# notu97/GS-SLAM-Analytica_Jacobian

Hardware: AMD Instinct MI355X
Metric: Gaussian-pixel interactions/sec (fwd+Jacobian), 640x480 (higher is better)
Workload: dtype f32; 1 GPU; cfg2: 50000 Gaussians (SH degree 3, 16 coeffs), 640x480; one step = one mapping window of 8 keyframes with distinct cameras: forward splat + analytical-Jacobian backward (dL/dmu, dL/dSigma->conic, per-Gaussian grads summed over the window, one dL/dtau per keyframe)

## Files before the change

gs-slam-analytica_jacobian_amd/csrc/api.hip:

```cpp
#include <stdarg.h>
#include <stdio.h>
#include <string.h>

#include <atomic>
#include <mutex>

#include "gsaj_common.h"
#include "loss_terms.h"

static thread_local char g_err[512] = "";

void gsaj_set_error(const char *fmt, ...) {
  va_list ap;
  va_start(ap, fmt);
  vsnprintf(g_err, sizeof(g_err), fmt, ap);
  va_end(ap);
}

struct ProfRec { int stage; hipEvent_t a, b; };
static std::mutex g_prof_mu;
static ProfRec *g_prof = nullptr;
static std::atomic<bool> g_prof_on{false};
static int g_prof_cap = 0;
static std::atomic<int> g_prof_n{0};
static thread_local int t_prof_open = -1;

void gsaj_prof_mark(int stage, int is_stop, hipStream_t s) {
  if (!g_prof_on.load(std::memory_order_acquire)) return;
  std::lock_guard<std::mutex> lk(g_prof_mu);
  if (!g_prof) return;
  if (!is_stop) {
    const int i = g_prof_n.fetch_add(1);
    if (i >= g_prof_cap) { g_prof_n.store(g_prof_cap); t_prof_open = -1; return; }
    t_prof_open = i;
    g_prof[i].stage = stage;
    (void)hipEventRecord(g_prof[i].a, s);
  } else if (t_prof_open >= 0 && t_prof_open < g_prof_cap) {
    (void)hipEventRecord(g_prof[t_prof_open].b, s);
    t_prof_open = -1;
  }
}

extern "C" {

int gsaj_profile_begin(int max_records) {
  std::lock_guard<std::mutex> lk(g_prof_mu);
  if (g_prof || max_records <= 0) {
    gsaj_set_error("gsaj_profile_begin: already active or bad size");
    return GSAJ_ERR_INVALID_ARGUMENT;
  }
  g_prof = new ProfRec[max_records];
  for (int i = 0; i < max_records; i++) {
    GSAJ_HIP_CHECK(hipEventCreate(&g_prof[i].a));
    GSAJ_HIP_CHECK(hipEventCreate(&g_prof[i].b));
  }
  g_prof_cap = max_records;
  g_prof_n.store(0);
  g_prof_on.store(true, std::memory_order_release);
  return GSAJ_OK;
}

int gsaj_profile_end(float *stage_ms, int *stage_launches) {
  if (!stage_ms || !stage_launches) {
    gsaj_set_error("gsaj_profile_end: null output");
    return GSAJ_ERR_INVALID_ARGUMENT;
  }
  g_prof_on.store(false, std::memory_order_release);
  GSAJ_HIP_CHECK(hipDeviceSynchronize());
  std::lock_guard<std::mutex> lk(g_prof_mu);
  if (!g_prof) {
    gsaj_set_error("gsaj_profile_end: not active");
    return GSAJ_ERR_INVALID_ARGUMENT;
  }
  for (int i = 0; i < ST_COUNT; i++) { stage_ms[i] = 0.f; stage_launches[i] = 0; }
  const int nrec = g_prof_n.load() < g_prof_cap ? g_prof_n.load() : g_prof_cap;
  for (int i = 0; i < nrec; i++) {
    float ms = 0.f;
    if (hipEventElapsedTime(&ms, g_prof[i].a, g_prof[i].b) == hipSuccess) {
      stage_ms[g_prof[i].stage] += ms;
      stage_launches[g_prof[i].stage] += 1;
    }
  }
  for (int i = 0; i < g_prof_cap; i++) { (void)hipEventDestroy(g_prof[i].a); (void)hipEventDestroy(g_prof[i].b); }
  delete[] g_prof;
  g_prof = nullptr;
  g_prof_cap = 0;
  g_prof_n.store(0);
  return GSAJ_OK;
}

const char *gsaj_last_error(void) { return g_err; }
int gsaj_version(void) { return 103; }

size_t gsaj_geom_workspace_bytes(int P) { return geom_carve(nullptr, (size_t)(P > 0 ? P : 0), nullptr) + 256; }
size_t gsaj_image_workspace_bytes(int W, int H) { return image_carve(nullptr, W, H, nullptr) + 256; }
size_t gsaj_binning_workspace_bytes(int R) {
  return bin_carve(nullptr, (size_t)(R > 0 ? R : 0), nullptr) + 256;
}

static char *align_base(void *p) { return reinterpret_cast<char *>(gsaj_align(reinterpret_cast<size_t>(p))); }

int gsaj_forward_preprocess(int P, int D, int M, int W, int H, const float *means3D, const float *shs,
                            const float *colors_precomp, const float *opacities, const float *scales,
                            float scale_modifier, const float *rotations, const float *cov3D_precomp,
                            const float *viewmatrix, const float *projmatrix, const float *campos, float tanfovx,
                            float tanfovy, int prefiltered, int *radii, int *n_touched, void *geom_ws, void *image_ws,
                            void *stream) {
  return gsaj_forward_preprocess_cap(P, D, M, W, H, means3D, shs, colors_precomp, opacities, scales, scale_modifier, rotations,
                                     cov3D_precomp, viewmatrix, projmatrix, campos, tanfovx, tanfovy, prefiltered, radii,
                                     n_touched, geom_ws, image_ws, 0, 0, stream);
}

int gsaj_forward_preprocess_cap(int P, int D, int M, int W, int H, const float *means3D, const float *shs,
                                const float *colors_precomp, const float *opacities, const float *scales,
                                float scale_modifier, const float *rotations, const float *cov3D_precomp,
                                const float *viewmatrix, const float *projmatrix, const float *campos, float tanfovx,
                                float tanfovy, int prefiltered, int *radii, int *n_touched, void *geom_ws, void *image_ws,
                                int capacity, int tile_list_capacity, void *stream) {
  if (P <= 0 || W <= 0 || H <= 0 || !means3D || !opacities || !viewmatrix || !projmatrix || !geom_ws || !image_ws ||
      !n_touched) {
    gsaj_set_error("gsaj_forward_preprocess: invalid argument (P=%d W=%d H=%d)", P, W, H);
    return GSAJ_ERR_INVALID_ARGUMENT;
  }
  if ((shs == nullptr) == (colors_precomp == nullptr)) {
    gsaj_set_error("Please provide excatly one of either SHs or precomputed colors!");
    return GSAJ_ERR_INVALID_ARGUMENT;
  }
  if (((scales == nullptr || rotations == nullptr) && cov3D_precomp == nullptr) ||
      ((scales != nullptr || rotations != nullptr) && cov3D_precomp != nullptr)) {
    gsaj_set_error("Please provide exactly one of either scale/rotation pair or precomputed 3D covariance!");
    return GSAJ_ERR_INVALID_ARGUMENT;
  }
  if (shs && (!campos || M <= 0 || D < 0 || (D + 1) * (D + 1) > M || D > 3)) {
    gsaj_set_error("gsaj_forward_preprocess: SH degree %d needs %d coefficients, got M=%d", D, (D + 1) * (D + 1), M);
    return GSAJ_ERR_INVALID_ARGUMENT;
  }
  GeomWS g;
  geom_carve(align_base(geom_ws), (size_t)P, &g);
  FwdParams p;
  p.P = P; p.D = D; p.M = M; p.W = W; p.H = H;
  p.means3D = means3D; p.shs = shs; p.colors_precomp = colors_precomp; p.opacities = opacities;
  p.scales = scales; p.rotations = rotations; p.cov3D_precomp = cov3D_precomp;
  p.viewmatrix = viewmatrix; p.projmatrix = projmatrix; p.campos = campos;
  p.scale_modifier = scale_modifier; p.tanfovx = tanfovx; p.tanfovy = tanfovy;
  p.focal_y = H / (2.0f * tanfovy);
  p.focal_x = W / (2.0f * tanfovx);
  p.prefiltered = prefiltered;
  p.grid_x = (W + TILE - 1) / TILE; p.grid_y = (H + TILE - 1) / TILE;
  p.capacity = capacity;
  p.sort_cap = (tile_list_capacity > 0 && tile_list_capacity < SORT_CAP) ? tile_list_capacity : SORT_CAP;
  p.views = 1;
  ImageWS im;
  image_carve(align_base(image_ws), W, H, &im);
  return launch_preprocess(p, radii ? radii : g.internal_radii, n_touched, g, im, ViewStrides{0, 0, 0}, (hipStream_t)stream);
}

int gsaj_forward_num_rendered(int W, int H, const void *image_ws, void *stream, int *num_rendered, int *max_tile_list) {
  if (W <= 0 || H <= 0 || !image_ws || !num_rendered) {
    gsaj_set_error("gsaj_forward_num_rendered: invalid argument");
    return GSAJ_ERR_INVALID_ARGUMENT;
  }
  ImageWS im;
  image_carve(align_base(const_cast<void *>(image_ws)), W, H, &im);
  uint32_t host[4] = {0, 0, 0, 0};
  GSAJ_HIP_CHECK(hipMemcpyAsync(host, im.counters, sizeof(host), hipMemcpyDeviceToHost, (hipStream_t)stream));
  GSAJ_HIP_CHECK(hipStreamSynchronize((hipStream_t)stream));
  *num_rendered = (int)host[0];
  if (max_tile_list) *max_tile_list = (int)host[2];
  if (host[1] & ERR_PREFILTERED) {
    gsaj_set_error("Point is filtered although prefiltered is set. This shouldn't happen!");
    return GSAJ_ERR_PREFILTERED_CULLED;
  }
  if (host[1] & ERR_INTERNAL) {
    gsaj_set_error("internal error: tile histogram total != instance total");
    return GSAJ_ERR_HIP;
  }
  if (host[1] & ERR_CAPACITY) {
    gsaj_set_error("async forward aborted: binning arena too small (R=%u, longest tile list=%u)", host[0], host[2]);
    return GSAJ_ERR_WORKSPACE_TOO_SMALL;
  }
  return GSAJ_OK;
}

int gsaj_forward_aborted_count(int W, int H, void *image_ws, void *stream, int *count) {
  if (W <= 0 || H <= 0 || !image_ws || !count) {
    gsaj_set_error("gsaj_forward_aborted_count: invalid argument");
    return GSAJ_ERR_INVALID_ARGUMENT;
  }
  ImageWS im;
  image_carve(align_base(image_ws), W, H, &im);
  uint32_t host = 0;
  GSAJ_HIP_CHECK(hipMemcpyAsync(&host, im.sticky, sizeof(host), hipMemcpyDeviceToHost, (hipStream_t)stream));
  GSAJ_HIP_CHECK(hipStreamSynchronize((hipStream_t)stream));
  *count = (int)host;
  if (host) GSAJ_HIP_CHECK(hipMemsetAsync(im.sticky, 0, sizeof(uint32_t), (hipStream_t)stream));
  return GSAJ_OK;
}

const uint32_t *gsaj_forward_abort_flag(int W, int H, void *image_ws) {
  if (W <= 0 || H <= 0 || !image_ws) {
    gsaj_set_error("gsaj_forward_abort_flag: invalid argument");
    return nullptr;
  }
  ImageWS im;
  image_carve(align_base(image_ws), W, H, &im);
  return im.counters + 4;
}

int gsaj_set_tile_band(int W, int H, void *image_ws, int tile_row_begin, int tile_row_end, void *stream) {
  const int gy = (H + TILE - 1) / TILE;
  if (W <= 0 || H <= 0 || !image_ws || tile_row_begin < 0 || tile_row_end < tile_row_begin || tile_row_end > gy || gy > 0xffff) {
    gsaj_set_error("gsaj_set_tile_band: rows [%d, %d) are not a band of the %d tile rows of a %dx%d frame", tile_row_begin,
                   tile_row_end, gy, W, H);
    return GSAJ_ERR_INVALID_ARGUMENT;
  }
  ImageWS im;
  image_carve(align_base(image_ws), W, H, &im);
  const bool whole = tile_row_begin == 0 && tile_row_end == gy;
  if (!whole && tile_row_end == 0) {
    gsaj_set_error("gsaj_set_tile_band: the empty band [0, 0) cannot be expressed; give an empty band as [b, b) with b > 0");
    return GSAJ_ERR_INVALID_ARGUMENT;
  }
  const uint32_t band = whole ? 0u : ((uint32_t)tile_row_begin | ((uint32_t)tile_row_end << 16));
  GSAJ_HIP_CHECK(hipMemsetD32Async(reinterpret_cast<hipDeviceptr_t>(im.sticky + 1), (int)band, 1, (hipStream_t)stream));
  GSAJ_HIP_CHECK(hipMemsetD32Async(reinterpret_cast<hipDeviceptr_t>(im.sticky + 2), (int)~band, 1, (hipStream_t)stream));
  return GSAJ_OK;
}

int gsaj_forward_render(int P, int R, int max_tile_list, int W, int H, const float *bg, const float *colors_precomp,
                        const int *radii,
                        void *geom_ws, void *binning_ws, size_t binning_ws_bytes, void *image_ws, float *out_color,
                        float *out_depth, float *out_opacity, int *n_touched, int flags, void *stream) {
  if (P <= 0 || R < 0 || W <= 0 || H <= 0 || !bg || !geom_ws || !binning_ws || !image_ws || !out_color || !out_depth ||
      !out_opacity || !n_touched) {
    gsaj_set_error("gsaj_forward_render: invalid argument");
    return GSAJ_ERR_INVALID_ARGUMENT;
  }
  const size_t need = gsaj_binning_workspace_bytes(R);
  if (binning_ws_bytes < need) {
    gsaj_set_error("binning workspace too small: have %zu bytes, need %zu for R=%d", binning_ws_bytes, need, R);
    return GSAJ_ERR_WORKSPACE_TOO_SMALL;
  }
  hipStream_t s = (hipStream_t)stream;
  GeomWS g;
  geom_carve(align_base(geom_ws), (size_t)P, &g);
  ImageWS im;
  image_carve(align_base(image_ws), W, H, &im);
  BinWS b;
  bin_carve(align_base(binning_ws), (size_t)R, &b);
  const int gx = (W + TILE - 1) / TILE, gy = (H + TILE - 1) / TILE;
  (void)colors_precomp;
  (void)radii;
  const int sort_cap = max_tile_list < 0 ? 128 : (max_tile_list > SORT_CAP ? SORT_CAP : max_tile_list);
  int rc;
  if ((rc = launch_tile_binning(P, sort_cap, (flags & GSAJ_FWD_RECORDS_FP16) ? 1 : 0, gx, gy, g, b, im, 1, ViewStrides{0, 0, 0}, s)) != GSAJ_OK) return rc;
  return launch_render_forward(P, W, H, gx, gy, bg, g, b, im, out_color, out_depth, out_opacity, n_touched, 1, ViewStrides{0, 0, 0}, s);
}

int gsaj_rasterize_forward(int P, int D, int M, const float *bg, int W, int H, const float *means3D, const float *shs,
                           const float *colors_precomp, const float *opacities, const float *scales,
                           float scale_modifier, const float *rotations, const float *cov3D_precomp,
                           const float *viewmatrix, const float *projmatrix, const float *campos, float tanfovx,
                           float tanfovy, int prefiltered, float *out_color, float *out_depth, float *out_opacity,
                           int *radii, int *n_touched, void *geom_ws, void *binning_ws, size_t binning_ws_bytes,
                           void *image_ws, int *num_rendered_out, int flags, void *stream) {
  int rc = gsaj_forward_preprocess(P, D, M, W, H, means3D, shs, colors_precomp, opacities, scales, scale_modifier,
                                   rotations, cov3D_precomp, viewmatrix, projmatrix, campos, tanfovx, tanfovy,
                                   prefiltered, radii, n_touched, geom_ws, image_ws, stream);
  if (rc != GSAJ_OK) return rc;
  int R = 0, max_tile = 0;
  rc = gsaj_forward_num_rendered(W, H, image_ws, stream, &R, &max_tile);
  if (num_rendered_out) *num_rendered_out = R;
  if (rc != GSAJ_OK) return rc;
  rc = gsaj_forward_render(P, R, max_tile, W, H, bg, colors_precomp, radii, geom_ws, binning_ws, binning_ws_bytes, image_ws,
                           out_color, out_depth, out_opacity, n_touched, flags, stream);
  return rc == GSAJ_OK ? R : rc;
}

static int forward_async_impl(int P, int D, int M, const float *bg, int W, int H, const float *means3D, const float *shs,
                              const float *colors_precomp, const float *opacities, const float *scales,
                              float scale_modifier, const float *rotations, const float *cov3D_precomp,
                              const float *viewmatrix, const float *projmatrix, const float *campos, float tanfovx,
                              float tanfovy, int prefiltered, float *out_color, float *out_depth, float *out_opacity,
                              int *radii, int *n_touched, void *geom_ws, void *binning_ws, size_t binning_ws_bytes,
                              int capacity, int tile_list_capacity, void *image_ws, int flags, void *stream, const FusedLoss *fl,
                              float *out_scalars) {
  if (capacity <= 0 || !binning_ws || !bg || !out_color || !out_depth || !out_opacity || !n_touched) {
    gsaj_set_error("gsaj_rasterize_forward_async: invalid argument");
    return GSAJ_ERR_INVALID_ARGUMENT;
  }
  if (binning_ws_bytes < gsaj_binning_workspace_bytes(capacity)) {
    gsaj_set_error("binning workspace smaller than gsaj_binning_workspace_bytes(capacity=%d)", capacity);
    return GSAJ_ERR_WORKSPACE_TOO_SMALL;
  }
  int rc = gsaj_forward_preprocess_cap(P, D, M, W, H, means3D, shs, colors_precomp, opacities, scales, scale_modifier,
                                       rotations, cov3D_precomp, viewmatrix, projmatrix, campos, tanfovx, tanfovy,
                                       prefiltered, radii, n_touched, geom_ws, image_ws, capacity, tile_list_capacity, stream);
  if (rc != GSAJ_OK) return rc;
  hipStream_t s = (hipStream_t)stream;
  GeomWS g;
  geom_carve(align_base(geom_ws), (size_t)P, &g);
  ImageWS im;
  image_carve(align_base(image_ws), W, H, &im);
  BinWS b;
  bin_carve(align_base(binning_ws), (size_t)capacity, &b);
  const int gx = (W + TILE - 1) / TILE, gy = (H + TILE - 1) / TILE;
  const int sort_cap = (tile_list_capacity > 0 && tile_list_capacity < SORT_CAP) ? tile_list_capacity : SORT_CAP;
  if ((rc = launch_tile_binning(P, sort_cap, (flags & GSAJ_FWD_RECORDS_FP16) ? 1 : 0, gx, gy, g, b, im, 1, ViewStrides{0, 0, 0}, s)) != GSAJ_OK) return rc;
  if ((rc = launch_render_forward(P, W, H, gx, gy, bg, g, b, im, out_color, out_depth, out_opacity, n_touched, 1, ViewStrides{0, 0, 0}, s, fl)) != GSAJ_OK) return rc;
  if (fl) return launch_loss_finalize(*fl, gsaj_fwd_loss_slots(W, H), W, H, im.counters + 4, out_scalars, s);
  return GSAJ_OK;
}

int gsaj_rasterize_forward_async(int P, int D, int M, const float *bg, int W, int H, const float *means3D, const float *shs,
                                 const float *colors_precomp, const float *opacities, const float *scales,
                                 float scale_modifier, const float *rotations, const float *cov3D_precomp,
                                 const float *viewmatrix, const float *projmatrix, const float *campos, float tanfovx,
                                 float tanfovy, int prefiltered, float *out_color, float *out_depth, float *out_opacity,
                                 int *radii, int *n_touched, void *geom_ws, void *binning_ws, size_t binning_ws_bytes,
                                 int capacity, int tile_list_capacity, void *image_ws, int flags, void *stream) {
  return forward_async_impl(P, D, M, bg, W, H, means3D, shs, colors_precomp, opacities, scales, scale_modifier, rotations, cov3D_precomp,
                            viewmatrix, projmatrix, campos, tanfovx, tanfovy, prefiltered, out_color, out_depth, out_opacity, radii,
                            n_touched, geom_ws, binning_ws, binning_ws_bytes, capacity, tile_list_capacity, image_ws, flags, stream,
                            nullptr, nullptr);
}

static int fused_loss_args(const char *who, int loss_flags, const float *gt_color, const float *gt_depth, const float *exposure_a,
                           const float *exposure_b) {
  const bool mono = loss_flags & GSAJ_LOSS_MONOCULAR, noexp = loss_flags & GSAJ_LOSS_NO_EXPOSURE;
  if ((loss_flags & GSAJ_LOSS_COMPUTE_LOSS) || !gt_color || (!mono && !gt_depth) || (!noexp && (!exposure_a || !exposure_b))) {
    gsaj_set_error("%s: invalid loss arguments (flags=%d; GSAJ_LOSS_COMPUTE_LOSS has no fused form)", who, loss_flags);
    return GSAJ_ERR_INVALID_ARGUMENT;
  }
  return GSAJ_OK;
}

size_t gsaj_fused_loss_workspace_bytes(int W, int H) { return (size_t)gsaj_fwd_loss_slots(W, H) * 4 * sizeof(float) + 256; }

int gsaj_rasterize_forward_loss(int P, int D, int M, const float *bg, int W, int H, const float *means3D, const float *shs,
                                const float *colors_precomp, const float *opacities, const float *scales, float scale_modifier,
                                const float *rotations, const float *cov3D_precomp, const float *viewmatrix,
                                const float *projmatrix, const float *campos, float tanfovx, float tanfovy, int prefiltered,
                                float *out_color, float *out_depth, float *out_opacity, int *radii, int *n_touched, void *geom_ws,
                                void *binning_ws, size_t binning_ws_bytes, int capacity, int tile_list_capacity, void *image_ws,
                                int flags, int loss_flags, float alpha, float rgb_boundary_threshold, const float *gt_color,
                                const float *gt_depth, const uint8_t *grad_mask, const float *exposure_a, const float *exposure_b,
                                float *out_scalars, void *loss_ws, void *stream) {
  int rc = fused_loss_args("gsaj_rasterize_forward_loss", loss_flags, gt_color, gt_depth, exposure_a, exposure_b);
  if (rc != GSAJ_OK) return rc;
  if (!out_scalars || !loss_ws) {
    gsaj_set_error("gsaj_rasterize_forward_loss: out_scalars and loss_ws are required");
    return GSAJ_ERR_INVALID_ARGUMENT;
  }
  FusedLoss fl{};
  fl.flags = loss_flags; fl.alpha = alpha; fl.rgb_thr = rgb_boundary_threshold;
  fl.gt_color = gt_color; fl.gt_depth = gt_depth; fl.grad_mask = grad_mask; fl.exp_a = exposure_a; fl.exp_b = exposure_b;
  fl.partials = reinterpret_cast<float *>(align_base(loss_ws));
  return forward_async_impl(P, D, M, bg, W, H, means3D, shs, colors_precomp, opacities, scales, scale_modifier, rotations, cov3D_precomp,
                            viewmatrix, projmatrix, campos, tanfovx, tanfovy, prefiltered, out_color, out_depth, out_opacity, radii,
                            n_touched, geom_ws, binning_ws, binning_ws_bytes, capacity, tile_list_capacity, image_ws, flags, stream, &fl,
                            out_scalars);
}

static int batch_workspaces(int K, int P, int capacity, int W, int H, void *geom_ws, void *binning_ws, size_t binning_ws_bytes,
                            void *image_ws, GeomWS *g, BinWS *b, ImageWS *im, ViewStrides *vs) {
  vs->geom = gsaj_geom_workspace_bytes(P);
  vs->image = gsaj_image_workspace_bytes(W, H);
  vs->bin = gsaj_binning_workspace_bytes(capacity);
  if (((uintptr_t)geom_ws | (uintptr_t)binning_ws | (uintptr_t)image_ws) & 255) {
    gsaj_set_error("batched entry points need 256-byte aligned workspaces");
    return GSAJ_ERR_INVALID_ARGUMENT;
  }
  if (binning_ws_bytes < vs->bin * (size_t)K) {
    gsaj_set_error("binning workspace smaller than K x gsaj_binning_workspace_bytes(capacity=%d)", capacity);
    return GSAJ_ERR_WORKSPACE_TOO_SMALL;
  }
  geom_carve(reinterpret_cast<char *>(geom_ws), (size_t)P, g);
  image_carve(reinterpret_cast<char *>(image_ws), W, H, im);
  bin_carve(reinterpret_cast<char *>(binning_ws), (size_t)capacity, b);
  return GSAJ_OK;
}

int gsaj_rasterize_forward_batch(int K, int P, int D, int M, const float *bg, int W, int H, const float *means3D, const float *shs,
                                 const float *colors_precomp, const float *opacities, const float *scales, float scale_modifier,
                                 const float *rotations, const float *cov3D_precomp, const float *viewmatrices,
                                 const float *projmatrices, const float *campos, float tanfovx, float tanfovy, int prefiltered,
                                 float *out_color, float *out_depth, float *out_opacity, int *radii, int *n_touched, void *geom_ws,
                                 void *binning_ws, size_t binning_ws_bytes, int capacity, int tile_list_capacity, void *image_ws,
                                 int flags, void *stream) {
  if (K <= 0 || P <= 0 || W <= 0 || H <= 0 || capacity <= 0 || !means3D || !opacities || !viewmatrices || !projmatrices || !bg ||
      !out_color || !out_depth || !out_opacity || !radii || !n_touched || !geom_ws || !binning_ws || !image_ws) {
    gsaj_set_error("gsaj_rasterize_forward_batch: invalid argument (K=%d P=%d W=%d H=%d capacity=%d)", K, P, W, H, capacity);
    return GSAJ_ERR_INVALID_ARGUMENT;
  }
  if ((shs == nullptr) == (colors_precomp == nullptr)) {
    gsaj_set_error("Please provide excatly one of either SHs or precomputed colors!");
    return GSAJ_ERR_INVALID_ARGUMENT;
  }
  if (((scales == nullptr || rotations == nullptr) && cov3D_precomp == nullptr) ||
      ((scales != nullptr || rotations != nullptr) && cov3D_precomp != nullptr)) {
    gsaj_set_error("Please provide exactly one of either scale/rotation pair or precomputed 3D covariance!");
    return GSAJ_ERR_INVALID_ARGUMENT;
  }
  if (shs && (!campos || M <= 0 || D < 0 || (D + 1) * (D + 1) > M || D > 3)) {
    gsaj_set_error("gsaj_rasterize_forward_batch: SH degree %d needs %d coefficients, got M=%d", D, (D + 1) * (D + 1), M);
    return GSAJ_ERR_INVALID_ARGUMENT;
  }
  GeomWS g; BinWS b; ImageWS im; ViewStrides vs;
  int rc = batch_workspaces(K, P, capacity, W, H, geom_ws, binning_ws, binning_ws_bytes, image_ws, &g, &b, &im, &vs);
  if (rc != GSAJ_OK) return rc;
  hipStream_t s = (hipStream_t)stream;
  FwdParams p;
  p.P = P; p.D = D; p.M = M; p.W = W; p.H = H;
  p.means3D = means3D; p.shs = shs; p.colors_precomp = colors_precomp; p.opacities = opacities;
  p.scales = scales; p.rotations = rotations; p.cov3D_precomp = cov3D_precomp;
  p.viewmatrix = viewmatrices; p.projmatrix = projmatrices; p.campos = campos;
  p.scale_modifier = scale_modifier; p.tanfovx = tanfovx; p.tanfovy = tanfovy;
  p.focal_y = H / (2.0f * tanfovy);
  p.focal_x = W / (2.0f * tanfovx);
  p.prefiltered = prefiltered;
  p.grid_x = (W + TILE - 1) / TILE; p.grid_y = (H + TILE - 1) / TILE;
  p.capacity = capacity;
  p.sort_cap = (tile_list_capacity > 0 && tile_list_capacity < SORT_CAP) ? tile_list_capacity : SORT_CAP;
  p.views = K;
  if ((rc = launch_preprocess(p, radii, n_touched, g, im, vs, s)) != GSAJ_OK) return rc;
  if ((rc = launch_tile_binning(P, p.sort_cap, (flags & GSAJ_FWD_RECORDS_FP16) ? 1 : 0, p.grid_x, p.grid_y, g, b, im, K, vs, s)) != GSAJ_OK)
    return rc;
  return launch_render_forward(P, W, H, p.grid_x, p.grid_y, bg, g, b, im, out_color, out_depth, out_opacity, n_touched, K, vs, s);
}

int gsaj_rasterize_backward_batch(int K, int P, int D, int M, int capacity, const float *bg, int W, int H, const float *means3D,
                                  const float *shs, const float *colors_precomp, const float *scales, float scale_modifier,
                                  const float *rotations, const float *cov3D_precomp, const float *viewmatrices,
                                  const float *projmatrices, const float *projmatrix_raw, const float *campos, float tanfovx,
                                  float tanfovy, const int *radii, void *geom_ws, void *binning_ws, void *image_ws,
                                  const float *dL_dpix, const float *dL_dpix_depth, float *dL_dmean2D, float *dL_dconic,
                                  float *dL_dopacity, float *dL_dcolor, float *dL_ddepth, float *dL_dmean3D, float *dL_dcov3D,
                                  float *dL_dsh, float *dL_dscale, float *dL_drot, float *dL_dtau, float *dL_dtau_sum, int flags,
                                  void *stream) {
  if (K <= 0 || P <= 0 || capacity <= 0 || W <= 0 || H <= 0 || !bg || !means3D || !viewmatrices || !projmatrices || !projmatrix_raw ||
      !radii || !geom_ws || !binning_ws || !image_ws || !dL_dpix || !dL_dpix_depth || !dL_dopacity || !dL_dmean3D || !dL_dcov3D ||
      !dL_dtau_sum) {
    gsaj_set_error("gsaj_rasterize_backward_batch: invalid argument");
    return GSAJ_ERR_INVALID_ARGUMENT;
  }
  if ((shs && (!dL_dsh || !campos)) || (scales && (!rotations || !dL_dscale || !dL_drot)) || (!scales && !cov3D_precomp)) {
    gsaj_set_error("gsaj_rasterize_backward_batch: missing gradient buffer for a provided input");
    return GSAJ_ERR_INVALID_ARGUMENT;
  }
  GeomWS g; BinWS b; ImageWS im; ViewStrides vs;
  int rc = batch_workspaces(K, P, capacity, W, H, geom_ws, binning_ws, gsaj_binning_workspace_bytes(capacity) * (size_t)K, image_ws,
                            &g, &b, &im, &vs);
  if (rc != GSAJ_OK) return rc;
  hipStream_t s = (hipStream_t)stream;
  const int gx = (W + TILE - 1) / TILE, gy = (H + TILE - 1) / TILE;
  const int fused = (flags & (GSAJ_BWD_ONLY_COMPOSITE | GSAJ_BWD_ONLY_CHAIN)) ? 0 : 1;
  if (!(flags & GSAJ_BWD_ONLY_CHAIN)) {
    if ((rc = launch_render_backward(capacity, W, H, gx, gy, bg, g, b, im, dL_dpix, dL_dpix_depth, K, vs, s)) != GSAJ_OK) return rc;
    if (!fused && (rc = launch_gather_sums(P, K, radii, g, b, im, vs, s)) != GSAJ_OK) return rc;
  }
  if (flags & GSAJ_BWD_ONLY_COMPOSITE) return GSAJ_OK;
  BwdParams p;
  p.P = P; p.D = D; p.M = M; p.W = W; p.H = H;
  p.means3D = means3D; p.shs = shs; p.scales = scales; p.rotations = rotations;
  p.cov3Ds = cov3D_precomp ? cov3D_precomp : g.cov3D;
  p.viewmatrix = viewmatrices; p.projmatrix = projmatrices; p.projmatrix_raw = projmatrix_raw; p.campos = campos;
  p.scale_modifier = scale_modifier; p.tanfovx = tanfovx; p.tanfovy = tanfovy;
  p.focal_y = H / (2.0f * tanfovy);
  p.focal_x = W / (2.0f * tanfovx);
  p.grid_x = gx; p.grid_y = gy;
  p.radii = radii;
  p.dL_dmean2D = dL_dmean2D; p.dL_dconic = dL_dconic; p.dL_dopacity = dL_dopacity; p.dL_dcolor = dL_dcolor;
  p.dL_ddepth = dL_ddepth; p.dL_dmean3D = dL_dmean3D; p.dL_dcov3D = dL_dcov3D; p.dL_dsh = dL_dsh;
  p.dL_dscale = dL_dscale; p.dL_drot = dL_drot; p.dL_dtau = dL_dtau; p.dL_dtau_sum = dL_dtau_sum;
  (void)colors_precomp;
  return launch_gaussian_backward_batch(p, K, g, b, im, vs, (flags & GSAJ_BWD_ACCUMULATE) ? 1 : 0, fused, s);
}

static int backward_impl(int P, int D, int M, int R, const float *bg, int W, int H, const float *means3D,
                         const float *shs, const float *colors_precomp, const float *scales, float scale_modifier,
                         const float *rotations, const float *cov3D_precomp, const float *viewmatrix,
                         const float *projmatrix, const float *projmatrix_raw, const float *campos, float tanfovx,
                         float tanfovy, const int *radii, void *geom_ws, void *binning_ws, void *image_ws,
                         const float *dL_dpix, const float *dL_dpix_depth, float *dL_dmean2D, float *dL_dconic,
                         float *dL_dopacity, float *dL_dcolor, float *dL_ddepth, float *dL_dmean3D,
                         float *dL_dcov3D, float *dL_dsh, float *dL_dscale, float *dL_drot, float *dL_dtau,
                         float *dL_dtau_sum, void *stream, const FusedLoss *fl) {
  const bool pose_only = !dL_dmean2D && !dL_dconic && !dL_dopacity && !dL_dcolor && !dL_ddepth && !dL_dmean3D && !dL_dcov3D &&
                         !dL_dsh && !dL_dscale && !dL_drot && dL_dtau_sum;
  if (P <= 0 || R < 0 || W <= 0 || H <= 0 || !bg || !means3D || !viewmatrix || !projmatrix || !projmatrix_raw ||
      !geom_ws || !binning_ws || !image_ws || (!fl && (!dL_dpix || !dL_dpix_depth)) ||
      (!pose_only && (!dL_dmean2D || !dL_dconic || !dL_dopacity || !dL_dcolor || !dL_ddepth || !dL_dmean3D || !dL_dcov3D))) {
    gsaj_set_error("gsaj_rasterize_backward: invalid argument");
    return GSAJ_ERR_INVALID_ARGUMENT;
  }
  if ((shs && ((!pose_only && !dL_dsh) || !campos)) || (scales && (!rotations || (!pose_only && (!dL_dscale || !dL_drot)))) ||
      (!scales && !cov3D_precomp)) {
    gsaj_set_error("gsaj_rasterize_backward: missing gradient buffer for a provided input");
    return GSAJ_ERR_INVALID_ARGUMENT;
  }
  hipStream_t s = (hipStream_t)stream;
  GeomWS g;
  geom_carve(align_base(geom_ws), (size_t)P, &g);
  ImageWS im;
  image_carve(align_base(image_ws), W, H, &im);
  BinWS b;
  bin_carve(align_base(binning_ws), (size_t)R, &b);
  const int gx = (W + TILE - 1) / TILE, gy = (H + TILE - 1) / TILE;
  int rc = launch_render_backward(R, W, H, gx, gy, bg, g, b, im, dL_dpix, dL_dpix_depth, 1, ViewStrides{0, 0, 0}, s, fl);
  if (rc != GSAJ_OK) return rc;
  BwdParams p;
  p.P = P; p.D = D; p.M = M; p.W = W; p.H = H;
  p.means3D = means3D; p.shs = shs; p.scales = scales; p.rotations = rotations;
  p.cov3Ds = cov3D_precomp ? cov3D_precomp : g.cov3D;
  p.viewmatrix = viewmatrix; p.projmatrix = projmatrix; p.projmatrix_raw = projmatrix_raw; p.campos = campos;
  p.scale_modifier = scale_modifier; p.tanfovx = tanfovx; p.tanfovy = tanfovy;
  p.focal_y = H / (2.0f * tanfovy);
  p.focal_x = W / (2.0f * tanfovx);
  p.grid_x = gx; p.grid_y = gy;
  p.radii = radii ? radii : g.internal_radii;
  p.dL_dmean2D = dL_dmean2D; p.dL_dconic = dL_dconic; p.dL_dopacity = dL_dopacity; p.dL_dcolor = dL_dcolor;
  p.dL_ddepth = dL_ddepth; p.dL_dmean3D = dL_dmean3D; p.dL_dcov3D = dL_dcov3D; p.dL_dsh = dL_dsh;
  p.dL_dscale = dL_dscale; p.dL_drot = dL_drot; p.dL_dtau = dL_dtau; p.dL_dtau_sum = dL_dtau_sum;
  (void)colors_precomp;
  return launch_gaussian_backward(p, g, b, im, s);
}

int gsaj_rasterize_backward(int P, int D, int M, int R, const float *bg, int W, int H, const float *means3D,
                            const float *shs, const float *colors_precomp, const float *scales, float scale_modifier,
                            const float *rotations, const float *cov3D_precomp, const float *viewmatrix,
                            const float *projmatrix, const float *projmatrix_raw, const float *campos, float tanfovx,
                            float tanfovy, const int *radii, void *geom_ws, void *binning_ws, void *image_ws,
                            const float *dL_dpix, const float *dL_dpix_depth, float *dL_dmean2D, float *dL_dconic,
                            float *dL_dopacity, float *dL_dcolor, float *dL_ddepth, float *dL_dmean3D,
                            float *dL_dcov3D, float *dL_dsh, float *dL_dscale, float *dL_drot, float *dL_dtau,
                            float *dL_dtau_sum, void *stream) {
  return backward_impl(P, D, M, R, bg, W, H, means3D, shs, colors_precomp, scales, scale_modifier, rotations, cov3D_precomp, viewmatrix,
                       projmatrix, projmatrix_raw, campos, tanfovx, tanfovy, radii, geom_ws, binning_ws, image_ws, dL_dpix, dL_dpix_depth,
                       dL_dmean2D, dL_dconic, dL_dopacity, dL_dcolor, dL_ddepth, dL_dmean3D, dL_dcov3D, dL_dsh, dL_dscale, dL_drot, dL_dtau,
                       dL_dtau_sum, stream, nullptr);
}

int gsaj_rasterize_backward_loss(int P, int D, int M, int R, const float *bg, int W, int H, const float *means3D, const float *shs,
                                 const float *colors_precomp, const float *scales, float scale_modifier, const float *rotations,
                                 const float *cov3D_precomp, const float *viewmatrix, const float *projmatrix,
                                 const float *projmatrix_raw, const float *campos, float tanfovx, float tanfovy, const int *radii,
                                 void *geom_ws, void *binning_ws, void *image_ws, int loss_flags, float alpha,
                                 float rgb_boundary_threshold, const float *color, const float *depth, const float *opacity,
                                 const float *gt_color, const float *gt_depth, const uint8_t *grad_mask, const float *exposure_a,
                                 const float *exposure_b, float *dL_dmean2D, float *dL_dconic, float *dL_dopacity, float *dL_dcolor,
                                 float *dL_ddepth, float *dL_dmean3D, float *dL_dcov3D, float *dL_dsh, float *dL_dscale,
                                 float *dL_drot, float *dL_dtau, float *dL_dtau_sum, void *stream) {
  int rc = fused_loss_args("gsaj_rasterize_backward_loss", loss_flags, gt_color, gt_depth, exposure_a, exposure_b);
  if (rc != GSAJ_OK) return rc;
  if (!color || !opacity || (!(loss_flags & GSAJ_LOSS_MONOCULAR) && !depth)) {
    gsaj_set_error("gsaj_rasterize_backward_loss: the forward's color / depth / opacity images are required");
    return GSAJ_ERR_INVALID_ARGUMENT;
  }
  FusedLoss fl{};
  fl.flags = loss_flags; fl.alpha = alpha; fl.rgb_thr = rgb_boundary_threshold;
  fl.gt_color = gt_color; fl.gt_depth = gt_depth; fl.grad_mask = grad_mask; fl.exp_a = exposure_a; fl.exp_b = exposure_b;
  fl.color = color; fl.depth = depth; fl.opacity = opacity;
  return backward_impl(P, D, M, R, bg, W, H, means3D, shs, colors_precomp, scales, scale_modifier, rotations, cov3D_precomp, viewmatrix,
                       projmatrix, projmatrix_raw, campos, tanfovx, tanfovy, radii, geom_ws, binning_ws, image_ws, nullptr, nullptr,
                       dL_dmean2D, dL_dconic, dL_dopacity, dL_dcolor, dL_ddepth, dL_dmean3D, dL_dcov3D, dL_dsh, dL_dscale, dL_drot, dL_dtau,
                       dL_dtau_sum, stream, &fl);
}

int gsaj_mark_visible(int P, const float *means3D, const float *viewmatrix, const float *projmatrix, uint8_t *present,
                      void *stream) {
  (void)projmatrix;
  if (P <= 0 || !means3D || !viewmatrix || !present) {
    gsaj_set_error("gsaj_mark_visible: invalid argument");
    return GSAJ_ERR_INVALID_ARGUMENT;
  }
  return launch_mark_visible(P, means3D, viewmatrix, present, (hipStream_t)stream);
}

int gsaj_debug_export(int P, int R, int W, int H, const void *geom_ws, const void *binning_ws, const void *image_ws,
                      float *means2D, float *depths, float *cov3D, float *conic_opacity, float *rgb, uint8_t *clamped,
                      uint32_t *tiles_touched, uint32_t *point_list, uint32_t *ranges, float *final_T,
                      uint32_t *n_contrib, void *stream) {
  hipStream_t s = (hipStream_t)stream;
  const size_t Pz = (size_t)P, N = (size_t)W * H;
  const size_t tiles = (size_t)((W + TILE - 1) / TILE) * ((H + TILE - 1) / TILE);
#define CP(dst, src, bytes) \
  if (dst) GSAJ_HIP_CHECK(hipMemcpyAsync(dst, src, bytes, hipMemcpyDeviceToDevice, s))
  if (geom_ws) {
    GeomWS g;
    geom_carve(align_base(const_cast<void *>(geom_ws)), Pz, &g);
#define CP2D(dst, src, width) \
  if (dst) GSAJ_HIP_CHECK(hipMemcpy2DAsync(dst, width, src, sizeof(float4) * REC_F4, width, Pz, hipMemcpyDeviceToDevice, s))
    CP2D(means2D, g.splat, sizeof(float2));
    CP2D(conic_opacity, g.splat + 1, sizeof(float4));
    CP2D(rgb, g.splat + 2, sizeof(float) * 3);
#undef CP2D
    CP(depths, g.depths, sizeof(float) * Pz);
    CP(cov3D, g.cov3D, sizeof(float) * 6 * Pz);
    CP(clamped, g.clamped, 3 * Pz);
    CP(tiles_touched, g.tiles_touched, sizeof(uint32_t) * Pz);
  }
  if (binning_ws && R > 0) {
    BinWS b;
    bin_carve(align_base(const_cast<void *>(binning_ws)), (size_t)R, &b);
    CP(point_list, b.point_list, sizeof(uint32_t) * (size_t)R);
  }
  if (image_ws) {
    ImageWS im;
    image_carve(align_base(const_cast<void *>(image_ws)), W, H, &im);
    CP(ranges, im.ranges, sizeof(uint2) * tiles);
    CP(final_T, im.final_T, sizeof(float) * N);
    CP(n_contrib, im.n_contrib, sizeof(uint32_t) * N);
  }
#undef CP
  return GSAJ_OK;
}

int gsaj_debug_export_view_sums(int P, const void *geom_ws, float *sums, void *stream) {
  if (P <= 0 || !geom_ws || !sums) {
    gsaj_set_error("gsaj_debug_export_view_sums: invalid argument");
    return GSAJ_ERR_INVALID_ARGUMENT;
  }
  GeomWS g;
  geom_carve(align_base(const_cast<void *>(geom_ws)), (size_t)P, &g);
  GSAJ_HIP_CHECK(hipMemcpyAsync(sums, g.gsum, sizeof(float4) * 3 * (size_t)P, hipMemcpyDeviceToDevice, (hipStream_t)stream));
  return GSAJ_OK;
}

int gsaj_debug_export_view_sums_gather(int P, int capacity, int W, int H, void *geom_ws, void *binning_ws, void *image_ws, float *sums,
                                       void *stream) {
  if (P <= 0 || capacity <= 0 || W <= 0 || H <= 0 || !geom_ws || !binning_ws || !image_ws || !sums) {
    gsaj_set_error("gsaj_debug_export_view_sums_gather: invalid argument");
    return GSAJ_ERR_INVALID_ARGUMENT;
  }
  GeomWS g; BinWS b; ImageWS im; ViewStrides vs;
  int rc = batch_workspaces(1, P, capacity, W, H, geom_ws, binning_ws, gsaj_binning_workspace_bytes(capacity), image_ws, &g, &b, &im, &vs);
  if (rc != GSAJ_OK) return rc;
  if ((rc = launch_gather_sums(P, 1, nullptr, g, b, im, vs, (hipStream_t)stream)) != GSAJ_OK) return rc;
  GSAJ_HIP_CHECK(hipMemcpyAsync(sums, g.gsum, sizeof(float4) * 3 * (size_t)P, hipMemcpyDeviceToDevice, (hipStream_t)stream));
  return GSAJ_OK;
}

}
```

gs-slam-analytica_jacobian_amd/csrc/gsaj_common.h:

```cpp
#pragma once
#include <hip/hip_runtime.h>
#include <stddef.h>
#include <stdint.h>

#include "../../include/gsaj.h"

#define GSAJ_WAVE 64
#define TILE GSAJ_TILE
#define TILE_PIXELS (TILE * TILE)
#define PRE_BLOCK 256
#define GB_BLOCK 64
#define REC_F4 3
#define IGRAD_F 12


static inline __host__ __device__ size_t gsaj_align(size_t x) { return (x + 255) & ~(size_t)255; }

struct GeomWS {
  float *depths;
  float *cov3D;
  uint8_t *clamped;
  uint32_t *tiles_touched;
  uint32_t *point_offsets;
  int *internal_radii;
  uint32_t *block_sums;
  float *tau_partials;
  float4 *splat;
  float4 *splat16;
  uint2 *scat;
  float4 *gsum;
};

static inline __host__ __device__ size_t geom_carve(char *base, size_t P, GeomWS *g) {
  size_t off = 0;
  size_t nblk = (P + PRE_BLOCK - 1) / PRE_BLOCK;
  if (nblk == 0) nblk = 1;
#define CARVE(field, type, count)                                \
  do {                                                           \
    if (g) g->field = reinterpret_cast<type *>(base + off);      \
    off += gsaj_align(sizeof(type) * (size_t)(count));           \
  } while (0)
  CARVE(depths, float, P);
  CARVE(cov3D, float, P * 6);
  CARVE(clamped, uint8_t, P * 3);
  CARVE(tiles_touched, uint32_t, P);
  CARVE(point_offsets, uint32_t, P);
  CARVE(internal_radii, int, P);
  CARVE(block_sums, uint32_t, nblk);
  CARVE(tau_partials, float, ((P + 31) / 32 + 1) * 8);
  CARVE(splat, float4, P * 3);
  CARVE(splat16, float4, P * 2);
  CARVE(scat, uint2, P);
  CARVE(gsum, float4, P * 3);
  return off;
}

#define TILE_REP 1
#define LDS_TILES_MAX 8192
#define SORT_CAP 16384
#define N_COUNTERS 64
#define ERR_PREFILTERED 1u
#define ERR_INTERNAL 2u
#define ERR_CAPACITY 4u
#define ERR_TILE_LIST 8u

struct ImageWS {
  float *final_T;
  uint32_t *n_contrib;
  uint2 *ranges;
  uint32_t *counters;
  uint32_t *tile_count;
  uint32_t *tile_cursor;
  uint32_t *tile_offset;
  uint32_t *sticky;
  uint32_t *tile_order;
  size_t zero_bytes;
};

static inline __host__ __device__ size_t image_carve(char *base, int W, int H, ImageWS *s) {
  size_t off = 0;
  size_t N = (size_t)W * H;
  size_t tiles = (size_t)((W + TILE - 1) / TILE) * ((H + TILE - 1) / TILE);
  ImageWS *g = s;
  CARVE(final_T, float, N);
  CARVE(n_contrib, uint32_t, N);
  CARVE(ranges, uint2, tiles);
  const size_t z0 = off;
  CARVE(counters, uint32_t, N_COUNTERS);
  CARVE(tile_count, uint32_t, tiles * TILE_REP);
  CARVE(tile_cursor, uint32_t, tiles * TILE_REP);
  if (g) g->zero_bytes = off - z0;
  CARVE(tile_offset, uint32_t, tiles * TILE_REP + 1);
  CARVE(sticky, uint32_t, 16);
  CARVE(tile_order, uint32_t, tiles);
  return off;
}

struct BinWS {
  uint64_t *keys_unsorted;
  uint64_t *keys;
  uint32_t *point_list;
  float4 *inst_grad;
  uint8_t *reached;
};

struct ViewStrides {
  size_t geom, image, bin;
};
#ifdef __HIPCC__
#include <type_traits>
template <typename T>
__device__ __forceinline__ T *gsaj_shift(T *p, size_t bytes) {
  typedef typename std::conditional<std::is_const<T>::value, const char, char>::type byte_t;
  return reinterpret_cast<T *>(reinterpret_cast<byte_t *>(p) + bytes);
}
__device__ __forceinline__ GeomWS geom_view(GeomWS g, size_t off) {
  g.depths = gsaj_shift(g.depths, off); g.cov3D = gsaj_shift(g.cov3D, off); g.clamped = gsaj_shift(g.clamped, off);
  g.tiles_touched = gsaj_shift(g.tiles_touched, off); g.point_offsets = gsaj_shift(g.point_offsets, off);
  g.internal_radii = gsaj_shift(g.internal_radii, off); g.block_sums = gsaj_shift(g.block_sums, off);
  g.tau_partials = gsaj_shift(g.tau_partials, off); g.splat = gsaj_shift(g.splat, off); g.gsum = gsaj_shift(g.gsum, off);
  g.splat16 = gsaj_shift(g.splat16, off); g.scat = gsaj_shift(g.scat, off);
  return g;
}
__device__ __forceinline__ ImageWS image_view(ImageWS m, size_t off) {
  m.final_T = gsaj_shift(m.final_T, off); m.n_contrib = gsaj_shift(m.n_contrib, off); m.ranges = gsaj_shift(m.ranges, off);
  m.counters = gsaj_shift(m.counters, off); m.tile_count = gsaj_shift(m.tile_count, off);
  m.tile_cursor = gsaj_shift(m.tile_cursor, off); m.tile_offset = gsaj_shift(m.tile_offset, off);
  m.sticky = gsaj_shift(m.sticky, off); m.tile_order = gsaj_shift(m.tile_order, off);
  return m;
}
#endif

static inline size_t bin_carve(char *base, size_t R, BinWS *g) {
  size_t off = 0;
  size_t Rn = R ? R : 1;
  CARVE(keys_unsorted, uint64_t, Rn);
  CARVE(keys, uint64_t, Rn);
  CARVE(point_list, uint32_t, Rn);
  CARVE(inst_grad, float4, Rn * REC_F4);
  CARVE(reached, uint8_t, Rn);
  return off;
}
#undef CARVE

void gsaj_set_error(const char *fmt, ...);
#define GSAJ_HIP_CHECK(expr)                                                          \
  do {                                                                                \
    hipError_t _e = (expr);                                                           \
    if (_e != hipSuccess) {                                                           \
      gsaj_set_error("%s failed: %s (%s:%d)", #expr, hipGetErrorString(_e), __FILE__, __LINE__); \
      return GSAJ_ERR_HIP;                                                            \
    }                                                                                 \
  } while (0)

enum GsajStage {
  ST_PREPROCESS = 0, ST_SCAN, ST_EMIT_KEYS, ST_SORT, ST_RANGES_RECORDS, ST_RENDER_FWD, ST_RENDER_BWD, ST_GAUSSIAN_BWD,
  ST_TAU_FINALIZE, ST_DENSE_BWD, ST_DENSE_REDUCE, ST_SCATTER, ST_TILE_SORT, ST_GATHER_SUMS, ST_COUNT
};
void gsaj_prof_mark(int stage, int is_stop, hipStream_t s);
struct GsajProfScope {
  int stage;
  hipStream_t s;
  GsajProfScope(int st, hipStream_t stream) : stage(st), s(stream) { gsaj_prof_mark(stage, 0, s); }
  ~GsajProfScope() { gsaj_prof_mark(stage, 1, s); }
};

struct FwdParams {
  int P, D, M, W, H;
  const float *means3D, *shs, *colors_precomp, *opacities, *scales, *rotations, *cov3D_precomp;
  const float *viewmatrix, *projmatrix, *campos;
  float scale_modifier, tanfovx, tanfovy, focal_x, focal_y;
  int prefiltered;
  int grid_x, grid_y;
  int capacity;
  int sort_cap;
  int bpw;
  int views;
};

int launch_preprocess(const FwdParams &p, int *radii, int *n_touched, const GeomWS &g, const ImageWS &im, ViewStrides vs,
                      hipStream_t s);
int launch_tile_binning(int P, int sort_cap, int rec16, int grid_x, int grid_y, const GeomWS &g, const BinWS &b, const ImageWS &im,
                        int views, ViewStrides vs, hipStream_t s);
struct FusedLoss;
int launch_render_forward(int P, int W, int H, int grid_x, int grid_y, const float *bg, const GeomWS &g, const BinWS &b,
                          const ImageWS &im, float *out_color, float *out_depth, float *out_opacity, int *n_touched, int views,
                          ViewStrides vs, hipStream_t s, const FusedLoss *fl = nullptr);
int gsaj_fwd_loss_slots(int W, int H);
int launch_loss_finalize(const FusedLoss &fl, int nslots, int W, int H, const uint32_t *aborted, float *out_scalars, hipStream_t s);
int launch_render_backward(int R, int W, int H, int grid_x, int grid_y, const float *bg, const GeomWS &g, const BinWS &b,
                           const ImageWS &im, const float *dL_dpix, const float *dL_dpix_depth, int views, ViewStrides vs,
                           hipStream_t s, const FusedLoss *fl = nullptr);
struct BwdParams {
  int P, D, M, W, H;
  const float *means3D, *shs, *scales, *rotations, *cov3Ds;
  const float *viewmatrix, *projmatrix, *projmatrix_raw, *campos;
  float scale_modifier, tanfovx, tanfovy, focal_x, focal_y;
  int grid_x, grid_y;
  const int *radii;
  float *dL_dmean2D, *dL_dconic, *dL_dopacity, *dL_dcolor, *dL_ddepth, *dL_dmean3D, *dL_dcov3D, *dL_dsh, *dL_dscale,
      *dL_drot, *dL_dtau, *dL_dtau_sum;
};
int launch_gaussian_backward(const BwdParams &p, const GeomWS &g, const BinWS &b, const ImageWS &im, hipStream_t s);
int launch_gather_sums(int P, int K, const int *radii, const GeomWS &g, const BinWS &b, const ImageWS &im, ViewStrides vs, hipStream_t s);
int launch_gaussian_backward_batch(const BwdParams &p, int K, const GeomWS &g, const BinWS &b, const ImageWS &im, ViewStrides vs,
                                   int accumulate, int gather, hipStream_t s);
int launch_mark_visible(int P, const float *means3D, const float *viewmatrix, uint8_t *present, hipStream_t s);
void launch_exclusive_scan_u32(int n, uint32_t *v, hipStream_t s);
int launch_select_rank_f32(int W, int H, const float *values, uint32_t rank, uint32_t *out_key, void *seed_ws, hipStream_t s);

#ifdef __HIPCC__
__device__ __forceinline__ float3 xform4x3(const float *m, float3 p) {
  return make_float3(m[0] * p.x + m[4] * p.y + m[8] * p.z + m[12], m[1] * p.x + m[5] * p.y + m[9] * p.z + m[13],
                     m[2] * p.x + m[6] * p.y + m[10] * p.z + m[14]);
}
__device__ __forceinline__ float4 xform4x4(const float *m, float3 p) {
  return make_float4(m[0] * p.x + m[4] * p.y + m[8] * p.z + m[12], m[1] * p.x + m[5] * p.y + m[9] * p.z + m[13],
                     m[2] * p.x + m[6] * p.y + m[10] * p.z + m[14], m[3] * p.x + m[7] * p.y + m[11] * p.z + m[15]);
}
__device__ __forceinline__ float ndc2pix(float v, int S) { return (float)((((double)v + 1.0) * (double)S - 1.0) * 0.5); }

__device__ __forceinline__ uint32_t gsaj_tile_band(const uint32_t *__restrict__ sticky) {
  const uint32_t band = sticky[1];
  return sticky[2] == ~band ? band : 0u;
}
__device__ __forceinline__ void tile_rect(float px, float py, int r, int gx, int gy, uint32_t band, int &x0, int &y0, int &x1,
                                          int &y1) {
  const int ylo = band ? (int)(band & 0xffffu) : 0, yhi = band ? min(gy, (int)(band >> 16)) : gy;
  x0 = min(gx, max(0, (int)((px - (float)r) / (float)TILE)));
  y0 = min(yhi, max(ylo, (int)((py - (float)r) / (float)TILE)));
  x1 = min(gx, max(0, (int)((px + (float)r + (float)(TILE - 1)) / (float)TILE)));
  y1 = min(yhi, max(ylo, (int)((py + (float)r + (float)(TILE - 1)) / (float)TILE)));
}
#define GSAJ_LOG2E 1.4426950408889634f
__device__ __forceinline__ float3 gsaj_prescale_conic(float a, float b, float c) {
  return make_float3((-0.5f * GSAJ_LOG2E) * a, -GSAJ_LOG2E * b, (-0.5f * GSAJ_LOG2E) * c);
}
__device__ __forceinline__ float gsaj_power2(float dx, float dy, float kx, float ky, float kz) {
  const float t = ky * dy;
  const float u = kz * dy;
  return __builtin_fmaf(dx, __builtin_fmaf(kx, dx, t), u * dy);
}
__device__ __forceinline__ float3 cross3(float3 a, float3 b) {
  return make_float3(a.y * b.z - a.z * b.y, a.z * b.x - a.x * b.z, a.x * b.y - a.y * b.x);
}
#endif

#define REC16_F4 2
#ifdef __HIPCC__
#include <hip/hip_fp16.h>
__device__ __forceinline__ uint32_t gsaj_pack_h2(float a, float b) {
  const __half2 h = __floats2half2_rn(a, b);
  return *reinterpret_cast<const uint32_t *>(&h);
}
__device__ __forceinline__ float2 gsaj_unpack_h2(uint32_t u) { return __half22float2(*reinterpret_cast<const __half2 *>(&u)); }
__device__ __forceinline__ void gsaj_load_row(const float4 *__restrict__ splat, const float4 *__restrict__ splat16, uint32_t id,
                                              bool rec16, float4 &q0, float4 &q1, float4 &q2) {
  if (!rec16) {
    const float4 *s = splat + (size_t)id * REC_F4;
    const float4 r0 = s[0], r1 = s[1], r2 = s[2];
    q0 = make_float4(r0.x, r0.y, r2.w, r0.w);
    q1 = r1;
    q2 = make_float4(r2.x, r2.y, r2.z, r0.z);
    return;
  }
  const float4 *s = splat16 + (size_t)id * REC16_F4;
  const float4 p0 = s[0], p1 = s[1];
  const float2 ab = gsaj_unpack_h2(__float_as_uint(p1.x)), co = gsaj_unpack_h2(__float_as_uint(p1.y));
  const float2 rg = gsaj_unpack_h2(__float_as_uint(p1.z)), bz = gsaj_unpack_h2(__float_as_uint(p1.w));
  q0 = p0;
  q1 = make_float4(ab.x, ab.y, co.x, co.y);
  q2 = make_float4(rg.x, rg.y, bz.x, 0.f);
}
#endif

#ifdef __HIPCC__
__device__ __forceinline__ float4 gsaj_load_f4_unaligned(const void *src) {
  typedef float f4u __attribute__((ext_vector_type(4), aligned(4)));
  const f4u v = *reinterpret_cast<const __attribute__((address_space(1))) f4u *>((unsigned long long)src);
  return make_float4(v.x, v.y, v.z, v.w);
}
__device__ __forceinline__ uint32_t gsaj_load_u32_global(const uint32_t *src) {
  return *reinterpret_cast<const __attribute__((address_space(1))) uint32_t *>((unsigned long long)src);
}
__device__ __forceinline__ uint4 gsaj_coherent_load_x4(const void *src) {
  uint4 v;
  asm volatile("global_load_dwordx4 %0, %1, off sc0 sc1\n\ts_waitcnt vmcnt(0)" : "=&v"(v) : "v"(src) : "memory");
  return v;
}
#endif

#ifdef GSAJ_BLOCK_TRACE
#define GSAJ_TRACE_MAX 65536
#define GSAJ_TRACE_DEFINE(NAME)                                                                               \
  __device__ unsigned long long g_trace_##NAME[4 * GSAJ_TRACE_MAX];                                           \
  extern "C" int gsaj_trace_read_##NAME(unsigned long long *host, int nwaves) {                               \
    return (int)hipMemcpyFromSymbol(host, HIP_SYMBOL(g_trace_##NAME), sizeof(unsigned long long) * 4 * nwaves); \
  }
#define GSAJ_TRACE_BEGIN(NAME)                                                                                \
  {                                                                                                           \
    const unsigned tw_ = (blockIdx.y * gridDim.x + blockIdx.x) * (blockDim.x >> 6) + (threadIdx.x >> 6);      \
    if ((threadIdx.x & 63) == 0 && tw_ < GSAJ_TRACE_MAX) {                                                    \
      g_trace_##NAME[4 * tw_ + 0] = wall_clock64();                                                           \
      g_trace_##NAME[4 * tw_ + 2] = __builtin_amdgcn_s_getreg((4) | (0 << 6) | (31 << 11));                   \
      g_trace_##NAME[4 * tw_ + 3] = __builtin_amdgcn_s_getreg((20) | (0 << 6) | (31 << 11));                  \
    }                                                                                                         \
  }
#define GSAJ_TRACE_END(NAME)                                                                                  \
  {                                                                                                           \
    const unsigned tw_ = (blockIdx.y * gridDim.x + blockIdx.x) * (blockDim.x >> 6) + (threadIdx.x >> 6);      \
    if ((threadIdx.x & 63) == 0 && tw_ < GSAJ_TRACE_MAX) g_trace_##NAME[4 * tw_ + 1] = wall_clock64();        \
  }
#else
#define GSAJ_TRACE_DEFINE(NAME)
#define GSAJ_TRACE_BEGIN(NAME)
#define GSAJ_TRACE_END(NAME)
#endif
```

gs-slam-analytica_jacobian_amd/csrc/render_bwd.hip:

```cpp
#include "gsaj_common.h"
#include "loss_terms.h"
#include "wave_reduce.h"

#define BWD_ROUND 48
#define SLOTS 8
#define WU_STRIDE 65
#define ACC_C 10
#define ACC_STRIDE (BWD_ROUND + 1)

GSAJ_TRACE_DEFINE(bwd)
GSAJ_TRACE_DEFINE(bwdph)
#ifdef GSAJ_BLOCK_TRACE
#define BWD_PH(i) { const unsigned long long now_ = wall_clock64(); ph_[i] += (unsigned)(now_ - pht_); pht_ = now_; }
#else
#define BWD_PH(i)
#endif

template <bool LOSS>
__global__ __launch_bounds__(256) __attribute__((amdgpu_waves_per_eu(5, 5))) void k_render_bwd(int W, int H, int gx, ImageWS im,
                                                    const uint32_t *__restrict__ point_list, GeomWS g,
                                                    const float *__restrict__ bg,
                                                    const float *__restrict__ dL_dpix,
                                                    const float *__restrict__ dL_dpix_depth,
                                                    float4 *__restrict__ inst_grad, uint8_t *__restrict__ reached, ViewStrides vs,
                                                    FusedLoss fl) {
  {
    const size_t view = blockIdx.y, HWv = (size_t)H * W;
    im = image_view(im, view * vs.image);
    point_list = gsaj_shift(point_list, view * vs.bin);
    g = geom_view(g, view * vs.geom);
    inst_grad = gsaj_shift(inst_grad, view * vs.bin);
    reached = gsaj_shift(reached, view * vs.bin);
    dL_dpix += view * 3 * HWv;
    dL_dpix_depth += view * HWv;
  }
  const uint2 *__restrict__ ranges = im.ranges;
  const float *__restrict__ final_T = im.final_T;
  const uint32_t *__restrict__ n_contrib = im.n_contrib;
  const uint32_t *__restrict__ counters = im.counters;
  __shared__ float4 rec[BWD_ROUND * REC_F4];
  __shared__ __attribute__((aligned(16))) float acc[4 * ACC_C * ACC_STRIDE];
  __shared__ float2 wu_all[4 * SLOTS * WU_STRIDE];
  __shared__ float4 seed_all[4 * 64];
  __shared__ uint32_t wave_max[4];
  __shared__ uint32_t blk_first[BWD_ROUND];
  if (counters[4]) return;
  GSAJ_TRACE_BEGIN(bwd)
  const int tid = threadIdx.x, wave = tid >> 6, lane = tid & 63;
  float2 *wu = wu_all + wave * SLOTS * WU_STRIDE;
  float4 *seed = seed_all + wave * 64;
  const int tile = __builtin_amdgcn_readfirstlane((int)min(im.tile_order[blockIdx.x], gridDim.x - 1));
  const int ty = tile / gx, tx = tile - ty * gx;
  const int px = tx * TILE + (wave & 1) * 8 + (lane & 7);
  const int py = ty * TILE + (wave >> 1) * 8 + (lane >> 3);
  const bool inside = px < W && py < H;
  const float pxf = (float)px, pyf = (float)py;
  const float qx0 = (float)(tx * TILE + (wave & 1) * 8), qy0 = (float)(ty * TILE + (wave >> 1) * 8);
  const uint2 range_v = ranges[tile];
  const uint2 range = make_uint2((uint32_t)__builtin_amdgcn_readfirstlane((int)range_v.x), (uint32_t)__builtin_amdgcn_readfirstlane((int)range_v.y));
  const size_t pid = (size_t)py * W + px, HW = (size_t)H * W;

  const float T_final = inside ? final_T[pid] : 0.f;
  float T = T_final;
  const uint32_t last = inside ? n_contrib[pid] : 0u;
  float gC0 = 0.f, gC1 = 0.f, gC2 = 0.f, gD = 0.f;
  if (inside) {
    if (LOSS) {
      const LossConsts L = loss_consts(fl.flags, fl.alpha, fl.rgb_thr, fl.exp_a, fl.exp_b, HW, 1.f);
      const bool mask = fl.grad_mask ? fl.grad_mask[pid] != 0 : true;
      const float gd = L.mono ? 0.f : fl.gt_depth[pid], d = L.mono ? 0.f : fl.depth[pid];
      const LossPixel o = loss_pixel(L, fl.gt_color[pid], fl.gt_color[HW + pid], fl.gt_color[2 * HW + pid], fl.color[pid], fl.color[HW + pid],
                                     fl.color[2 * HW + pid], fl.opacity[pid], mask, gd, d);
      gC0 = o.gC0; gC1 = o.gC1; gC2 = o.gC2; gD = o.gD;
    } else {
      gC0 = dL_dpix[pid];
      gC1 = dL_dpix[HW + pid];
      gC2 = dL_dpix[2 * HW + pid];
      gD = dL_dpix_depth[pid];
    }
  }
  seed[lane] = make_float4(gC0, gC1, gC2, gD);
  const float Tf_bg = T_final * (bg[0] * gC0 + bg[1] * gC1 + bg[2] * gC2);
  const float ddelx_dx = 0.5f * W, ddely_dy = 0.5f * H;

  uint32_t wmax = last;
#pragma unroll
  for (int o = 32; o > 0; o >>= 1) wmax = max(wmax, (uint32_t)__shfl_xor((int)wmax, o));
  if (lane == 0) wave_max[wave] = wmax;
  __syncthreads();
  const uint32_t bmax = max(max(wave_max[0], wave_max[1]), max(wave_max[2], wave_max[3]));

  float accS = 0.f;

  const int p2_slot = lane & (SLOTS - 1), p2_row = lane >> 3;
  const float p2_py = qy0 + (float)p2_row;

  uint32_t hi = (uint32_t)__builtin_amdgcn_readfirstlane((int)(range.x + bmax));
  const bool rec16 = counters[7] != 0u;
  const int part = __builtin_amdgcn_readfirstlane(wave), e = lane;
  auto round_lo = [&](uint32_t h) { return (h - range.x > BWD_ROUND) ? h - BWD_ROUND : range.x; };
  auto load_id = [&](uint32_t l, uint32_t h) -> uint32_t {
    const bool has = e < BWD_ROUND && l + (uint32_t)e < h;
    const uint32_t v = gsaj_load_u32_global(point_list + (has ? l + (uint32_t)e : range.x));
    return has ? v : 0xffffffffu;
  };
  const char *piece_base;
  uint32_t piece_stride;
  if (part == 3) piece_base = reinterpret_cast<const char *>(g.block_sums), piece_stride = 0u;
  else if (!rec16) piece_base = reinterpret_cast<const char *>(g.splat + part), piece_stride = 16u * REC_F4;
  else if (part < 2) piece_base = reinterpret_cast<const char *>(g.splat16 + part), piece_stride = 16u * REC16_F4;
  else piece_base = reinterpret_cast<const char *>(g.scat), piece_stride = 8u;
  auto load_piece = [&](uint32_t id) -> float4 {
    const uint32_t i = id != 0xffffffffu ? id : 0u;
    const size_t off = piece_stride ? (size_t)i * piece_stride : (size_t)(i / PRE_BLOCK) * 4u;
    return gsaj_load_f4_unaligned(piece_base + off);
  };
  uint32_t id_cur = 0xffffffffu, id_nxt = 0xffffffffu;
  float4 piece = make_float4(0.f, 0.f, 0.f, 0.f);
  if (hi > range.x) {
    const uint32_t lo0 = round_lo(hi);
    id_cur = load_id(lo0, hi);
    id_nxt = load_id(round_lo(lo0), lo0);
    piece = load_piece(id_cur);
  }

#ifdef GSAJ_BLOCK_TRACE
  unsigned ph_[7] = {0u, 0u, 0u, 0u, 0u, 0u, 0u};
  unsigned tr_flushes = 0u, tr_slots = 0u;
  unsigned long long pht_ = wall_clock64();
#endif
  while (hi > range.x) {
    BWD_PH(6)
    const uint32_t lo = round_lo(hi);
    const int n = (int)(hi - lo);
    if (e < n) {
      int e_ = e;
      asm volatile("" : "+v"(e_));
      const int e = e_;
      if (part == 3) {
        blk_first[e] = __float_as_uint(piece.x);
      } else if (!rec16) {
        if (part == 1) {
          const float3 kq = gsaj_prescale_conic(piece.x, piece.y, piece.z);
          rec[e * REC_F4 + 1] = make_float4(kq.x, kq.y, kq.z, piece.w);
        } else {
          rec[e * REC_F4 + part] = piece;
        }
      } else {
        float *r = reinterpret_cast<float *>(rec + e * REC_F4);
        if (part == 0) {
          r[0] = piece.x, r[1] = piece.y, r[3] = piece.w, r[11] = piece.z;
        } else if (part == 1) {
          const float2 ab = gsaj_unpack_h2(__float_as_uint(piece.x)), co = gsaj_unpack_h2(__float_as_uint(piece.y));
          const float2 rg = gsaj_unpack_h2(__float_as_uint(piece.z)), bz = gsaj_unpack_h2(__float_as_uint(piece.w));
          const float3 kq = gsaj_prescale_conic(ab.x, ab.y, co.x);
          rec[e * REC_F4 + 1] = make_float4(kq.x, kq.y, kq.z, co.y);
          r[8] = rg.x, r[9] = rg.y, r[10] = bz.x;
        } else if (part == 2) {
          const uint32_t sx = __float_as_uint(piece.x), sy = __float_as_uint(piece.y);
          const uint32_t x0 = sx & 0xffffu, y0 = sy & 0xffffu, w = (sx >> 16) - x0;
          r[2] = __uint_as_float(x0 | (y0 << 10) | (w << 20));
        }
      }
    }
    {
      const uint32_t lo2 = round_lo(lo);
      id_cur = id_nxt;
      id_nxt = load_id(round_lo(lo2), lo2);
      piece = load_piece(id_cur);
    }
    {
      float4 *z = reinterpret_cast<float4 *>(acc);
      for (int i = tid; i < 4 * ACC_C * ACC_STRIDE / 4; i += 256) z[i] = make_float4(0.f, 0.f, 0.f, 0.f);
    }
    BWD_PH(0)
    __syncthreads();
    BWD_PH(1)

    const uint32_t first_idx = (uint32_t)__builtin_amdgcn_readfirstlane((int)(lo - range.x));
    if (wmax > first_idx) {
      bool rel = false;
      if (lane < n && first_idx + (uint32_t)lane < wmax) {
        const float4 q0 = rec[lane * REC_F4 + 0];
        const float4 q1 = rec[lane * REC_F4 + 1];
        rel = quadrant_relevant(q0.x, q0.y, (-2.0f / GSAJ_LOG2E) * q1.x, (-1.0f / GSAJ_LOG2E) * q1.y, (-2.0f / GSAJ_LOG2E) * q1.z, q1.w, qx0, qy0);
      }
      unsigned long long todo = __builtin_amdgcn_ballot_w64(rel);
      int nslot = 0;
      unsigned long long slot_pack = 0ull;

      auto flush = [&]() {
#ifdef GSAJ_BLOCK_TRACE
        tr_flushes++;
        tr_slots += (unsigned)nslot;
#endif
        const int j = (int)((slot_pack >> (8 * p2_slot)) & 0xffull);
        const float4 e0 = rec[j * REC_F4 + 0];
        float4 e1 = rec[j * REC_F4 + 1];
        e1.x *= -2.0f / GSAJ_LOG2E; e1.y *= -1.0f / GSAJ_LOG2E; e1.z *= -2.0f / GSAJ_LOG2E;
        const float ax0 = e0.x - qx0, dy = e0.y - p2_py;
        float m0 = 0.f, swdx = 0.f, swdx2 = 0.f, u0 = 0.f, u1 = 0.f, u2 = 0.f, u3 = 0.f;
#pragma unroll
        for (int it = 0; it < 8; it++) {
          const int pix = p2_row * 8 + it;
          const float2 q = wu[p2_slot * WU_STRIDE + pix];
          const float4 sd = seed[pix];
          const float dx = ax0 - (float)it;
          const float wd = q.x * dx;
          m0 += q.x;
          swdx += wd;
          swdx2 = __builtin_fmaf(wd, dx, swdx2);
          u0 += q.y * sd.x;
          u1 += q.y * sd.y;
          u2 += q.y * sd.z;
          u3 += q.y * sd.w;
        }
        const float swdy = dy * m0;
        float v[10];
        v[0] = -(e1.x * swdx + e1.y * swdy) * ddelx_dx;
        v[1] = -(e1.z * swdy + e1.y * swdx) * ddely_dy;
        v[2] = -0.5f * swdx2;
        v[3] = -0.5f * (dy * swdx);
        v[4] = -0.5f * (dy * swdy);
        v[5] = m0 * __builtin_amdgcn_rcpf(e1.w);
        v[6] = u0; v[7] = u1; v[8] = u2; v[9] = u3;
        const float w0 = merge32(v[0], v[1]), w1 = merge32(v[2], v[3]), w2 = merge32(v[4], v[5]), w3 = merge32(v[6], v[7]),
                    w4 = merge32(v[8], v[9]);
        float x0 = merge16(w0, w1), x1 = merge16(w2, w3), x2 = merge16(w4, w4);
        x0 = dpp_add<0x128>(x0);
        x1 = dpp_add<0x128>(x1);
        x2 = dpp_add<0x128>(x2);
        if (p2_slot < nslot && (lane & 8) == 0) {
          const int r = lane >> 4;
          const int k = ((r & 1) << 1) | (r >> 1);
          float *a = acc + wave * ACC_C * ACC_STRIDE + j;
          a[k * ACC_STRIDE] = x0;
          a[(4 + k) * ACC_STRIDE] = x1;
          if ((r & 1) == 0) a[(8 + (r >> 1)) * ACC_STRIDE] = x2;
        }
        nslot = 0;
        slot_pack = 0ull;
      };

      if (todo != 0ull) {
        int jj = 63 - __builtin_clzll(todo);
        todo &= ~(1ull << jj);
        float2 q01 = reinterpret_cast<const float2 *>(rec)[jj * (REC_F4 * 2)];
        float4 k = rec[jj * REC_F4 + 1], c = rec[jj * REC_F4 + 2];
        while (true) {
          const int j = jj;
          const uint32_t idx = first_idx + (uint32_t)j;
          const bool more = todo != 0ull;
          if (more) {
            jj = 63 - __builtin_clzll(todo);
            todo &= ~(1ull << jj);
          }
          const float dx = q01.x - pxf, dy = q01.y - pyf;
          const float p2 = gsaj_power2(dx, dy, k.x, k.y, k.z);
          const float oG = k.w * __builtin_amdgcn_exp2f(p2);
          q01 = reinterpret_cast<const float2 *>(rec)[jj * (REC_F4 * 2)];
          k = rec[jj * REC_F4 + 1];
          const bool valid = idx < last && p2 <= 0.0f && oG >= (1.0f / 255.0f);
          float cg = __builtin_fmaf(c.x, gC0, __builtin_fmaf(c.y, gC1, __builtin_fmaf(c.z, gC2, c.w * gD)));
          asm volatile("" : "+v"(cg));
          c = rec[jj * REC_F4 + 2];
          if (__builtin_amdgcn_ballot_w64(valid) != 0ull) {
            const float oGm = valid ? oG : 0.f;
            float alpha;
            asm("v_min_f32 %0, 0x3f7d70a4, %1" : "=v"(alpha) : "v"(oGm));
            const float inv1ma = __builtin_amdgcn_rcpf(1.f - alpha);
            T = T * inv1ma;
            asm volatile("" : "+v"(T));
            const float dd = cg - accS;
            const float dL_dalpha = dd * T - Tf_bg * inv1ma;
            accS += alpha * dd;
            float w_ = dL_dalpha * oGm;
            asm volatile("" : "+v"(w_));
            wu[nslot * WU_STRIDE + lane] = make_float2(w_, alpha * T);
            slot_pack |= (unsigned long long)j << (8 * nslot);
            nslot++;
            if (nslot == SLOTS) flush();
          }
          if (!more) break;
        }
        if (nslot > 0) flush();
      }
    }
    BWD_PH(2)
    __syncthreads();
    BWD_PH(3)
    if (part < 3 && e < n) {
      float t[4];
#pragma unroll
      for (int c = 0; c < 4; c++) {
        const float *a = acc + min(part * 4 + c, ACC_C - 1) * ACC_STRIDE + e;
        t[c] = ((a[0] + a[ACC_C * ACC_STRIDE]) + a[2 * ACC_C * ACC_STRIDE]) + a[3 * ACC_C * ACC_STRIDE];
      }
      if (part == 2) t[2] = t[3] = 0.f;
      const float4 q0 = rec[e * REC_F4 + 0];
      const uint32_t rp = __float_as_uint(q0.z);
      const uint32_t x0 = rp & 1023u, y0 = (rp >> 10) & 1023u, w = rp >> 20;
      const uint32_t emit = blk_first[e] + __float_as_uint(q0.w) + ((uint32_t)ty - y0) * w + ((uint32_t)tx - x0);
      inst_grad[(size_t)emit * REC_F4 + part] = make_float4(t[0], t[1], t[2], t[3]);
      if (part == 0) reached[emit] = 1;
    }
    BWD_PH(4)
    __syncthreads();
    BWD_PH(5)
    hi = lo;
  }
#ifdef GSAJ_BLOCK_TRACE
  {
    const unsigned tw_ = (blockIdx.y * gridDim.x + blockIdx.x) * 4 + (threadIdx.x >> 6);
    if ((threadIdx.x & 63) == 0 && tw_ < GSAJ_TRACE_MAX) {
      g_trace_bwdph[4 * tw_ + 0] = ((unsigned long long)ph_[0] << 32) | ph_[1];
      g_trace_bwdph[4 * tw_ + 1] = ((unsigned long long)ph_[2] << 32) | ph_[3];
      g_trace_bwdph[4 * tw_ + 2] = ((unsigned long long)ph_[4] << 32) | ph_[5];
      g_trace_bwdph[4 * tw_ + 3] = ph_[6] | ((unsigned long long)tr_flushes << 32) | ((unsigned long long)tr_slots << 44);
    }
  }
#endif
  GSAJ_TRACE_END(bwd)
}

int launch_render_backward(int R, int W, int H, int grid_x, int grid_y, const float *bg, const GeomWS &g, const BinWS &b,
                           const ImageWS &im, const float *dL_dpix, const float *dL_dpix_depth, int views, ViewStrides vs,
                           hipStream_t s, const FusedLoss *fl) {
  if (R <= 0) return GSAJ_OK;
  {
    GsajProfScope ps(ST_RENDER_BWD, s);
    if (fl)
      hipLaunchKernelGGL(k_render_bwd<true>, dim3(grid_x * grid_y, 1), dim3(256), 0, s, W, H, grid_x, im, b.point_list, g, bg, dL_dpix,
                         dL_dpix_depth, b.inst_grad, b.reached, vs, *fl);
    else
      hipLaunchKernelGGL(k_render_bwd<false>, dim3(grid_x * grid_y, views), dim3(256), 0, s, W, H, grid_x, im, b.point_list, g, bg, dL_dpix,
                         dL_dpix_depth, b.inst_grad, b.reached, vs, FusedLoss{});
  }
  GSAJ_HIP_CHECK(hipGetLastError());
  return GSAJ_OK;
}
```

gs-slam-analytica_jacobian_amd/csrc/render_fwd.hip:

```cpp
#include "gsaj_common.h"
#include "loss_terms.h"
#include "wave_reduce.h"

#define FWD_CHUNK 64
#define FWD_PAD 8
#define FWD_PAIR_F4 6
typedef float v2f __attribute__((ext_vector_type(2)));

#ifndef GSAJ_FWD_THREADS
#define GSAJ_FWD_THREADS 64
#endif
#define FWD_WAVES (GSAJ_FWD_THREADS / 64)

GSAJ_TRACE_DEFINE(fwd)

template <bool LOSS>
__global__ __launch_bounds__(GSAJ_FWD_THREADS) __attribute__((amdgpu_waves_per_eu(5, 8))) void k_render_fwd(int W, int H, int gx, int tiles, int P, ImageWS im,
                                                    const float4 *__restrict__ splat, const float4 *__restrict__ splat16,
                                                    const float *__restrict__ bg,
                                                    float *__restrict__ out_color, float *__restrict__ out_depth,
                                                    float *__restrict__ out_opacity, int *__restrict__ n_touched,
                                                    const uint32_t *__restrict__ point_list, ViewStrides vs, FusedLoss fl) {
  {
    const size_t view = blockIdx.y, HWv = (size_t)H * W;
    im = image_view(im, view * vs.image);
    splat = gsaj_shift(splat, view * vs.geom);
    splat16 = gsaj_shift(splat16, view * vs.geom);
    point_list = gsaj_shift(point_list, view * vs.bin);
    out_color += view * 3 * HWv;
    out_depth += view * HWv;
    out_opacity += view * HWv;
    n_touched += view * (size_t)P;
  }
  const uint2 *__restrict__ ranges = im.ranges;
  float *__restrict__ final_T = im.final_T;
  uint32_t *__restrict__ n_contrib = im.n_contrib;
  uint32_t *__restrict__ counters = im.counters;
  __shared__ float4 rec_all[FWD_WAVES * ((FWD_CHUNK + FWD_PAD) / 2) * FWD_PAIR_F4];
  if (counters[4]) return;
  GSAJ_TRACE_BEGIN(fwd)
  const int tid = threadIdx.x, lane = tid & 63;
#if FWD_WAVES == 1
  const int wave = ((int)blockIdx.x >> 3) & 3;
  const int rank = ((int)blockIdx.x >> 5) * 8 + ((int)blockIdx.x & 7);
  if (rank >= tiles) {
    if (LOSS && lane == 0) reinterpret_cast<float4 *>(fl.partials)[blockIdx.x] = make_float4(0.f, 0.f, 0.f, 0.f);
    return;
  }
  const int tile = (int)min(im.tile_order[rank], (uint32_t)(tiles - 1));
  float4 *rec = rec_all;
#else
  const int wave = tid >> 6;
  const int tile = (int)min(im.tile_order[blockIdx.x], (uint32_t)(tiles - 1));
  float4 *rec = rec_all + wave * ((FWD_CHUNK + FWD_PAD) / 2) * FWD_PAIR_F4;
#endif
  const int ty = tile / gx, tx = tile - ty * gx;
  const int px = tx * TILE + (wave & 1) * 8 + (lane & 7);
  const int py = ty * TILE + (wave >> 1) * 8 + (lane >> 3);
  const bool inside = px < W && py < H;
  const float pxf = (float)px, pyf = (float)py;
  const float qx0 = (float)(tx * TILE + (wave & 1) * 8), qy0 = (float)(ty * TILE + (wave >> 1) * 8);
  const uint2 range = ranges[tile];

  bool done = !inside;
  float T = 1.0f;
  uint32_t last = 0;
  bool counting = true;

  v2f Crg = {0.f, 0.f}, Cbd = {0.f, 0.f};
  const v2f px2 = {pxf, pxf}, py2 = {pyf, pyf};
  auto composite2 = [&](const float4 p0, const float4 p1, const float4 p2, const float4 cA, const float4 cB, const float2 pos,
                        float &T_afterA) {
    const v2f dx = v2f{p0.x, p0.y} - px2, dy = v2f{p0.z, p0.w} - py2;
    const v2f t = v2f{p1.z, p1.w} * dy;
    const v2f u = v2f{p2.x, p2.y} * dy;
    const v2f pw = __builtin_elementwise_fma(dx, __builtin_elementwise_fma(v2f{p1.x, p1.y}, dx, t), u * dy);
    const v2f oe = v2f{p2.z, p2.w} * v2f{__builtin_amdgcn_exp2f(pw.x), __builtin_amdgcn_exp2f(pw.y)};
    {
      const float alpha0 = fminf(0.99f, oe.x);
      bool ok = !done && pw.x <= 0.0f && alpha0 >= (1.0f / 255.0f);
      const float tA = __builtin_fmaf(-alpha0, T, T);
      const bool sat = ok && tA < 0.0001f;
      done = done || sat;
      ok = ok && !sat;
      const float w = ok ? alpha0 * T : 0.f;
      const v2f w2 = {w, w};
      Crg = __builtin_elementwise_fma(v2f{cA.x, cA.y}, w2, Crg);
      Cbd = __builtin_elementwise_fma(v2f{cA.z, cA.w}, w2, Cbd);
      T = ok ? tA : T;
      last = ok ? __float_as_uint(pos.x) : last;
      T_afterA = T;
    }
    {
      const float alpha0 = fminf(0.99f, oe.y);
      bool ok = !done && pw.y <= 0.0f && alpha0 >= (1.0f / 255.0f);
      const float tB = __builtin_fmaf(-alpha0, T, T);
      const bool sat = ok && tB < 0.0001f;
      done = done || sat;
      ok = ok && !sat;
      const float w = ok ? alpha0 * T : 0.f;
      const v2f w2 = {w, w};
      Crg = __builtin_elementwise_fma(v2f{cB.x, cB.y}, w2, Crg);
      Cbd = __builtin_elementwise_fma(v2f{cB.z, cB.w}, w2, Cbd);
      T = ok ? tB : T;
      last = ok ? __float_as_uint(pos.y) : last;
    }
  };

  if (__builtin_amdgcn_ballot_w64(!done) != 0ull && range.x < range.y) {
    float4 q0, q1, q2;
    uint32_t id_cur = 0u, id_nxt = 0u;
    const bool rec16 = counters[7] != 0u;
    auto fetch_id = [&](uint32_t base) {
      if (base + (uint32_t)lane < range.y) id_nxt = point_list[base + lane];
    };
    auto fetch_row = [&](uint32_t base) {
      id_cur = id_nxt;
      if (base + (uint32_t)lane < range.y) gsaj_load_row(splat, splat16, id_nxt, rec16, q0, q1, q2);
    };
    float *recf = reinterpret_cast<float *>(rec);
    for (int i = lane; i < ((FWD_CHUNK + FWD_PAD) / 2) * FWD_PAIR_F4; i += 64) rec[i] = make_float4(0.f, 0.f, 0.f, 0.f);
    auto put = [&](int s, float x, float y, float kx, float ky, float kz, float o, float4 c, uint32_t pos, uint32_t id) {
      const int h = s & 1, pb = (s >> 1) * FWD_PAIR_F4;
      float *f = recf + pb * 4 + h;
      f[0] = x; f[2] = y; f[4] = kx; f[6] = ky; f[8] = kz; f[10] = o;
      rec[pb + 3 + h] = c;
      f[20] = __uint_as_float(pos); f[22] = __uint_as_float(id);
    };
    fetch_id(range.x);
    fetch_row(range.x);
    fetch_id(range.x + FWD_CHUNK);
    for (uint32_t base = range.x; base < range.y; base += FWD_CHUNK) {
      const int m = min((uint32_t)FWD_CHUNK, range.y - base);
      bool rel = false;
      const uint32_t id_here = id_cur;
      if (lane < m) rel = quadrant_relevant(q0.x, q0.y, q1.x, q1.y, q1.z, q1.w, qx0, qy0);
      const unsigned long long todo = __builtin_amdgcn_ballot_w64(rel);
      const int nrel = __popcll(todo);
      __builtin_amdgcn_wave_barrier();
      if (rel) {
        const int slot = __builtin_amdgcn_mbcnt_hi((uint32_t)(todo >> 32), __builtin_amdgcn_mbcnt_lo((uint32_t)todo, 0u));
        const float3 k = gsaj_prescale_conic(q1.x, q1.y, q1.z);
        put(slot, q0.x, q0.y, k.x, k.y, k.z, q1.w, make_float4(q2.x, q2.y, q2.z, q0.z), base - range.x + (uint32_t)lane + 1u, id_here);
      }
      if (lane < FWD_PAD) recf[((nrel + lane) >> 1) * FWD_PAIR_F4 * 4 + 10 + ((nrel + lane) & 1)] = 0.f;
      fetch_row(base + FWD_CHUNK);
      fetch_id(base + 2 * FWD_CHUNK);
      __builtin_amdgcn_fence(__ATOMIC_RELEASE, "wavefront");
      __builtin_amdgcn_wave_barrier();
      __builtin_amdgcn_fence(__ATOMIC_ACQUIRE, "wavefront");
      uint32_t cnt4 = 0u;
      bool wave_done = false;
      const float2 *rec2 = reinterpret_cast<const float2 *>(rec);
      float4 a0 = rec[0], a1 = rec[1], a2 = rec[2], a3 = rec[3], a4 = rec[4];
      float2 a5 = rec2[10];
      for (int i = 0; i < nrel; i += 4) {
        const int pb = (i >> 1) * FWD_PAIR_F4;
        const float4 c0 = rec[pb + 6], c1 = rec[pb + 7], c2 = rec[pb + 8], c3 = rec[pb + 9], c4 = rec[pb + 10];
        const float2 c5 = rec2[(pb + 11) * 2];
        uint32_t pack = 0u;
        {
          const float T0 = T;
          float Ta;
          composite2(a0, a1, a2, a3, a4, a5, Ta);
          if (counting) {
            const unsigned long long hB = __builtin_amdgcn_ballot_w64(T > 0.5f);
            const uint32_t nA = (uint32_t)__popcll(__builtin_amdgcn_ballot_w64(Ta > 0.5f) & __builtin_amdgcn_ballot_w64(Ta < T0));
            const uint32_t nB = (uint32_t)__popcll(hB & __builtin_amdgcn_ballot_w64(T < Ta));
            pack = nA | (nB << 8);
            counting = hB != 0ull;
          }
        }
        asm volatile("" : "+v"(T), "+v"(last), "+v"(Crg), "+v"(Cbd) : : "memory");
        a0 = rec[pb + 12], a1 = rec[pb + 13], a2 = rec[pb + 14], a3 = rec[pb + 15], a4 = rec[pb + 16];
        a5 = rec2[(pb + 17) * 2];
        {
          const float T0 = T;
          float Tc;
          composite2(c0, c1, c2, c3, c4, c5, Tc);
          if (counting) {
            const unsigned long long hD = __builtin_amdgcn_ballot_w64(T > 0.5f);
            const uint32_t nC = (uint32_t)__popcll(__builtin_amdgcn_ballot_w64(Tc > 0.5f) & __builtin_amdgcn_ballot_w64(Tc < T0));
            const uint32_t nD = (uint32_t)__popcll(hD & __builtin_amdgcn_ballot_w64(T < Tc));
            pack |= (nC << 16) | (nD << 24);
            counting = hD != 0ull;
          }
        }
        cnt4 = ((lane >> 2) == (i >> 2)) ? pack : cnt4;
        if (__builtin_amdgcn_ballot_w64(!done) == 0ull) {
          wave_done = true;
          break;
        }
      }
      const int cnt = (int)((cnt4 >> (8 * (lane & 3))) & 0xffu);
      if (lane < nrel && cnt > 0) {
        const uint32_t id = __float_as_uint(recf[(lane >> 1) * FWD_PAIR_F4 * 4 + 22 + (lane & 1)]);
        atomicAdd(&n_touched[id], cnt);
      }
      __builtin_amdgcn_wave_barrier();
      if (wave_done) break;
    }
  }

  const float Cr = Crg.x, Cg = Crg.y, Cb = Cbd.x, Dp = Cbd.y;
  if (inside) {
    const size_t pid = (size_t)py * W + px;
    const size_t HW = (size_t)H * W;
    final_T[pid] = T;
    n_contrib[pid] = last;
    out_color[pid] = Cr + T * bg[0];
    out_color[HW + pid] = Cg + T * bg[1];
    out_color[2 * HW + pid] = Cb + T * bg[2];
    out_depth[pid] = Dp;
    out_opacity[pid] = 1.f - T;
  }
  if (LOSS) {
    float s4[4] = {0.f, 0.f, 0.f, 0.f};
    if (inside) {
      const size_t pid = (size_t)py * W + px, HW = (size_t)H * W;
      const LossConsts L = loss_consts(fl.flags, fl.alpha, fl.rgb_thr, fl.exp_a, fl.exp_b, HW, 1.f);
      const bool mask = fl.grad_mask ? fl.grad_mask[pid] != 0 : true;
      const float gd = L.mono ? 0.f : fl.gt_depth[pid];
      const LossPixel o = loss_pixel(L, fl.gt_color[pid], fl.gt_color[HW + pid], fl.gt_color[2 * HW + pid], Cr + T * bg[0], Cg + T * bg[1],
                                     Cb + T * bg[2], 1.f - T, mask, gd, Dp);
      s4[0] = o.s_rgb; s4[1] = o.s_d; s4[2] = o.s_a; s4[3] = o.s_b;
    }
#pragma unroll
    for (int c = 0; c < 4; c++) {
#pragma unroll
      for (int o2 = 32; o2 > 0; o2 >>= 1) s4[c] += __shfl_xor(s4[c], o2);
    }
    if (lane == 0) reinterpret_cast<float4 *>(fl.partials)[blockIdx.x] = make_float4(s4[0], s4[1], s4[2], s4[3]);
  }
  GSAJ_TRACE_END(fwd)
}

int gsaj_fwd_loss_slots(int W, int H) {
  const int tiles = ((W + TILE - 1) / TILE) * ((H + TILE - 1) / TILE);
  return FWD_WAVES == 1 ? ((tiles + 7) / 8) * 32 : tiles;
}

int launch_render_forward(int P, int W, int H, int grid_x, int grid_y, const float *bg, const GeomWS &g, const BinWS &b,
                          const ImageWS &im, float *out_color, float *out_depth, float *out_opacity, int *n_touched, int views,
                          ViewStrides vs, hipStream_t s, const FusedLoss *fl) {
  static_assert(FWD_WAVES == 1, "the loss-fused epilogue writes one partial per wave-sized workgroup");
  {
    GsajProfScope ps(ST_RENDER_FWD, s);
    const int tiles = grid_x * grid_y;
    const unsigned nblk = FWD_WAVES == 1 ? (unsigned)((tiles + 7) / 8) * 32u : (unsigned)tiles;
    if (fl)
      hipLaunchKernelGGL(k_render_fwd<true>, dim3(nblk, 1), dim3(GSAJ_FWD_THREADS), 0, s, W, H, grid_x, tiles, P, im, g.splat, g.splat16, bg,
                         out_color, out_depth, out_opacity, n_touched, b.point_list, vs, *fl);
    else
      hipLaunchKernelGGL(k_render_fwd<false>, dim3(nblk, views), dim3(GSAJ_FWD_THREADS), 0, s, W, H, grid_x, tiles, P, im, g.splat, g.splat16,
                         bg, out_color, out_depth, out_opacity, n_touched, b.point_list, vs, FusedLoss{});
  }
  GSAJ_HIP_CHECK(hipGetLastError());
  return GSAJ_OK;
}
```

gs-slam-analytica_jacobian_amd/gsaj/_lib.py:

```python
import ctypes
import os
import subprocess

_HERE = os.path.dirname(os.path.abspath(__file__))
PKG_ROOT = os.path.dirname(_HERE)
CSRC = os.path.join(PKG_ROOT, "csrc")
LIB_PATH = os.environ.get("GSAJ_LIB_PATH") or os.path.join(PKG_ROOT, "lib", "libgsaj_hip.so")
HEADER = os.path.join(os.path.dirname(PKG_ROOT), "include", "gsaj.h")

c_int, c_float, c_double, c_size_t, c_void_p = ctypes.c_int, ctypes.c_float, ctypes.c_double, ctypes.c_size_t, ctypes.c_void_p
P = c_void_p

SIGNATURES = {
    "gsaj_last_error": (ctypes.c_char_p, []),
    "gsaj_version": (c_int, []),
    "gsaj_geom_workspace_bytes": (c_size_t, [c_int]),
    "gsaj_image_workspace_bytes": (c_size_t, [c_int, c_int]),
    "gsaj_binning_workspace_bytes": (c_size_t, [c_int]),
    "gsaj_forward_preprocess": (c_int, [c_int] * 5 + [P, P, P, P, P, c_float, P, P, P, P, P, c_float, c_float, c_int, P, P, P, P, P]),
    "gsaj_forward_num_rendered": (c_int, [c_int, c_int, P, P, ctypes.POINTER(c_int), ctypes.POINTER(c_int)]),
    "gsaj_forward_render": (c_int, [c_int] * 5 + [P, P, P, P, P, c_size_t, P, P, P, P, P, c_int, P]),
    "gsaj_rasterize_forward": (c_int, [c_int, c_int, c_int, P, c_int, c_int, P, P, P, P, P, c_float, P, P, P, P, P,
                                       c_float, c_float, c_int, P, P, P, P, P, P, P, c_size_t, P,
                                       ctypes.POINTER(c_int), c_int, P]),
    "gsaj_rasterize_forward_async": (c_int, [c_int, c_int, c_int, P, c_int, c_int, P, P, P, P, P, c_float, P, P, P, P, P,
                                             c_float, c_float, c_int, P, P, P, P, P, P, P, c_size_t, c_int, c_int, P, c_int, P]),
    "gsaj_rasterize_forward_batch": (c_int, [c_int, c_int, c_int, c_int, P, c_int, c_int, P, P, P, P, P, c_float, P, P, P, P, P,
                                             c_float, c_float, c_int, P, P, P, P, P, P, P, c_size_t, c_int, c_int, P, c_int, P]),
    "gsaj_rasterize_backward_batch": (c_int, [c_int, c_int, c_int, c_int, c_int, P, c_int, c_int, P, P, P, P, c_float, P, P, P, P,
                                              P, P, c_float, c_float, P, P, P, P, P, P] + [P] * 12 + [c_int, P]),
    "gsaj_fused_loss_workspace_bytes": (c_size_t, [c_int, c_int]),
    "gsaj_rasterize_forward_loss": (c_int, [c_int, c_int, c_int, P, c_int, c_int, P, P, P, P, P, c_float, P, P, P, P, P,
                                            c_float, c_float, c_int, P, P, P, P, P, P, P, c_size_t, c_int, c_int, P, c_int,
                                            c_int, c_float, c_float, P, P, P, P, P, P, P, P]),
    "gsaj_rasterize_backward_loss": (c_int, [c_int, c_int, c_int, c_int, P, c_int, c_int, P, P, P, P, c_float, P, P, P, P, P, P,
                                             c_float, c_float, P, P, P, P, c_int, c_float, c_float, P, P, P, P, P, P, P, P] + [P] * 12 + [P]),
    "gsaj_forward_aborted_count": (c_int, [c_int, c_int, P, P, ctypes.POINTER(c_int)]),
    "gsaj_set_tile_band": (c_int, [c_int, c_int, P, c_int, c_int, P]),
    "gsaj_forward_preprocess_cap": (c_int, [c_int] * 5 + [P, P, P, P, P, c_float, P, P, P, P, P, c_float, c_float, c_int, P, P,
                                            P, P, c_int, c_int, P]),
    "gsaj_rasterize_backward": (c_int, [c_int, c_int, c_int, c_int, P, c_int, c_int, P, P, P, P, c_float, P, P, P, P, P, P,
                                        c_float, c_float, P, P, P, P, P, P] + [P] * 12 + [P]),
    "gsaj_mark_visible": (c_int, [c_int, P, P, P, P, P]),
    "gsaj_debug_export": (c_int, [c_int] * 4 + [P] * 3 + [P] * 11 + [P]),
    "gsaj_debug_export_view_sums": (c_int, [c_int, P, P, P]),
    "gsaj_debug_export_view_sums_gather": (c_int, [c_int, c_int, c_int, c_int, P, P, P, P, P]),
    "gsaj_profile_begin": (c_int, [c_int]),
    "gsaj_profile_end": (c_int, [P, P]),
    "gsaj_dense_workspace_bytes": (c_size_t, [c_int, c_int, c_int]),
    "gsaj_dense_backward": (c_int, [c_int, c_int, c_int] + [P] * 7 + [P] * 4 + [P, c_int, P, P]),
    "gsaj_dense_project_workspace_bytes": (c_size_t, [c_int]),
    "gsaj_dense_project": (c_int, [c_int] * 5 + [P] * 6 + [c_double, c_double] + [P] * 6 + [P, P]),
    "gsaj_dense_render": (c_int, [c_int, c_int, c_int] + [P] * 5 + [P, P, P]),
    "gsaj_pose_jacobians": (c_int, [c_int, P, P, P, c_double, c_double, c_int, c_int, P, P, P]),
    "gsaj_dense_tau": (c_int, [c_int, c_int, c_int] + [P] * 11 + [P, P, P]),
    "gsaj_dist2_workspace_bytes": (c_size_t, [c_int]),
    "gsaj_dist2": (c_int, [c_int, P, P, P, P]),
    "gsaj_debug_dist2_order": (c_int, [c_int, P, P, P, P]),
    "gsaj_pose_state_floats": (c_int, []),
    "gsaj_pose_adam_step": (c_int, [P, P] + [c_float] * 8 + [P, P, P, P]),
    "gsaj_pose_adam_step_batch": (c_int, [c_int, P, P, P] + [c_float] * 8 + [P, P, P, c_size_t, P]),
    "gsaj_forward_abort_flag": (c_void_p, [c_int, c_int, P]),
    "gsaj_loss_workspace_bytes": (c_size_t, [c_int, c_int]),
    "gsaj_densification_stats": (c_int, [c_int, c_int] + [P] * 7 + [P]),
    "gsaj_isotropic_workspace_bytes": (c_size_t, [c_int]),
    "gsaj_isotropic_loss": (c_int, [c_int, c_int, c_float, P, P, c_int, P, P, P]),
    "gsaj_loss_seeds": (c_int, [c_int, c_int, c_int, c_float, c_float] + [P] * 8 + [P] * 4 + [P, P]),
    "gsaj_loss_seeds_batch": (c_int, [c_int] + [c_int, c_int, c_int, c_float, c_float] + [P] * 8 + [P] * 4 + [P, P]),
    "gsaj_ssim_workspace_bytes": (c_size_t, [c_int] * 4),
    "gsaj_ssim_forward": (c_int, [c_int] * 4 + [P] * 6),
    "gsaj_ssim_backward": (c_int, [c_int] * 4 + [P] * 6),
    "gsaj_refine_loss_workspace_bytes": (c_size_t, [c_int, c_int]),
    "gsaj_refine_loss_seeds": (c_int, [c_int, c_int, c_float] + [P] * 6),
    "gsaj_seed_workspace_bytes": (c_size_t, [c_int, c_int]),
    "gsaj_depth_stats": (c_int, [c_int, c_int, P, P, c_float, P, P, c_float, P, P, P, P]),
    "gsaj_keyframe_depth_prior": (c_int, [c_int, c_int, P, P, P, c_float, P, P, P, P, P]),
    "gsaj_seed_select": (c_int, [c_int, c_int, P, P, c_float, c_float, c_double, ctypes.c_uint32, P, P]),
    "gsaj_seed_count": (c_int, [P, P, ctypes.POINTER(c_int), ctypes.POINTER(c_int)]),
    "gsaj_debug_seed_pixels": (c_int, [c_int, c_int, c_int, P, P, P]),
    "gsaj_seed_gaussians": (c_int, [c_int, c_int, c_int, P, P, P, P] + [c_double] * 4 + [c_float, c_int, c_int, c_int] + [P] * 6 + [P, P, P]),
    "gsaj_grad_mask_workspace_bytes": (c_size_t, [c_int, c_int]),
    "gsaj_grad_intensity": (c_int, [c_int, c_int, P, P, P]),
    "gsaj_grad_mask": (c_int, [c_int, c_int, P, c_float, c_int, P, P, P, P]),
    "gsaj_covis_pack": (c_int, [c_int, c_int, P, ctypes.POINTER(c_int), ctypes.c_uint32, P, P]),
    "gsaj_covis_query": (c_int, [c_int, P, P, c_int, ctypes.c_uint32, P, P]),
    "gsaj_covis_prune_mask": (c_int, [c_int, P, ctypes.c_uint32, P, c_int, c_int, P, P, P, P]),
}

_lib = None


def build(verbose=False):
    cmd = ["make", "-C", CSRC, "-j8"]
    if not verbose:
        cmd.append("-s")
    subprocess.check_call(cmd)
    return LIB_PATH


def load():
    global _lib
    if _lib is not None:
        return _lib
    if not os.path.exists(LIB_PATH):
        raise ImportError(
            "libgsaj_hip.so is missing (%s). Build the HIP extension first: "
            "`python __graft_entry__.py` or `make -C %s`. There is no CPU fallback." % (LIB_PATH, CSRC))
    import torch
    lib = ctypes.CDLL(LIB_PATH)
    for name, (res, args) in SIGNATURES.items():
        fn = getattr(lib, name)
        fn.restype = res
        fn.argtypes = args
    _lib = lib
    return lib


class GsajError(RuntimeError):
    pass


def check(rc, what):
    if rc < 0:
        msg = load().gsaj_last_error().decode("utf-8", "replace")
        if rc == -1:
            raise Exception(msg or ("%s: invalid argument" % what))
        raise GsajError("%s failed (%d): %s" % (what, rc, msg))
    return rc
```

gs-slam-analytica_jacobian_amd/gsaj/rasterizer.py:

```python
import ctypes
import os

import torch

from . import _lib

_F32 = torch.float32
FORCE_CHUNKED_SORT = bool(int(__import__("os").environ.get("GSAJ_FORCE_CHUNKED_SORT", "0")))
SORT_CAP = 16384


def _ptr(t):
    if t is None or t.numel() == 0:
        return None
    return t.data_ptr()


def _prep(t, device, name):
    if t is None or t.numel() == 0:
        return None
    if t.device != device:
        t = t.to(device)
    if t.dtype != _F32:
        t = t.to(_F32)
    return t.contiguous()


def _stream(device):
    return torch.cuda.current_stream(device).cuda_stream


def _require_cuda(t, what):
    if not t.is_cuda:
        raise RuntimeError("%s must live on the GPU (HIP device): libgsaj_hip has no CPU path" % what)


def rasterize_gaussians(background, means3D, colors, opacity, scales, rotations, scale_modifier, cov3D_precomp,
                        viewmatrix, projmatrix, projmatrix_raw, tan_fovx, tan_fovy, image_height, image_width, sh,
                        degree, campos, prefiltered, debug, record_bits=32):
    lib = _lib.load()
    if means3D.ndim != 2 or means3D.shape[1] != 3:
        raise RuntimeError("means3D must have dimensions (num_points, 3)")
    _require_cuda(means3D, "means3D")
    dev = means3D.device
    P, H, W = means3D.shape[0], int(image_height), int(image_width)
    f = dict(device=dev, dtype=_F32)
    out_color = torch.zeros((3, H, W), **f)
    out_depth = torch.zeros((1, H, W), **f)
    out_opacity = torch.zeros((1, H, W), **f)
    radii = torch.zeros((P,), device=dev, dtype=torch.int32)
    n_touched = torch.zeros((P,), device=dev, dtype=torch.int32)
    byte = dict(device=dev, dtype=torch.uint8)
    if P == 0:
        e = torch.empty(0, **byte)
        return 0, out_color, radii, e, e.clone(), e.clone(), out_depth, out_opacity, n_touched

    means3D = _prep(means3D, dev, "means3D")
    colors = _prep(colors, dev, "colors")
    opacity = _prep(opacity, dev, "opacity")
    scales = _prep(scales, dev, "scales")
    rotations = _prep(rotations, dev, "rotations")
    cov3D_precomp = _prep(cov3D_precomp, dev, "cov3D")
    sh = _prep(sh, dev, "sh")
    background = _prep(background, dev, "bg")
    viewmatrix = _prep(viewmatrix, dev, "viewmatrix")
    projmatrix = _prep(projmatrix, dev, "projmatrix")
    campos = _prep(campos, dev, "campos")
    M = 0 if sh is None else sh.shape[1]

    geom = torch.empty(lib.gsaj_geom_workspace_bytes(P), **byte)
    img = torch.empty(lib.gsaj_image_workspace_bytes(W, H), **byte)
    st = _stream(dev)
    with torch.cuda.device(dev):
        _lib.check(lib.gsaj_forward_preprocess(
            P, int(degree), M, W, H, _ptr(means3D), _ptr(sh), _ptr(colors), _ptr(opacity), _ptr(scales),
            float(scale_modifier), _ptr(rotations), _ptr(cov3D_precomp), _ptr(viewmatrix), _ptr(projmatrix),
            _ptr(campos), float(tan_fovx), float(tan_fovy), int(bool(prefiltered)), radii.data_ptr(),
            n_touched.data_ptr(), geom.data_ptr(), img.data_ptr(), st), "gsaj_forward_preprocess")
        R, mt = ctypes.c_int(0), ctypes.c_int(0)
        _lib.check(lib.gsaj_forward_num_rendered(W, H, img.data_ptr(), st, ctypes.byref(R), ctypes.byref(mt)),
                   "gsaj_forward_num_rendered")
        R = R.value
        nbytes = lib.gsaj_binning_workspace_bytes(R)
        binning = torch.empty(nbytes, **byte)
        _lib.check(lib.gsaj_forward_render(
            P, R, -1 if FORCE_CHUNKED_SORT else mt.value, W, H, _ptr(background), _ptr(colors), radii.data_ptr(), geom.data_ptr(), binning.data_ptr(), nbytes,
            img.data_ptr(), out_color.data_ptr(), out_depth.data_ptr(), out_opacity.data_ptr(), n_touched.data_ptr(),
            _fwd_flags(record_bits), st), "gsaj_forward_render")
        if debug:
            torch.cuda.synchronize(dev)
    return R, out_color, radii, geom, binning, img, out_depth, out_opacity, n_touched


def rasterize_gaussians_backward(background, means3D, radii, colors, scales, rotations, scale_modifier, cov3D_precomp,
                                 viewmatrix, projmatrix, projmatrix_raw, tan_fovx, tan_fovy, dL_dout_color,
                                 dL_dout_depths, sh, degree, campos, geomBuffer, R, binningBuffer, imageBuffer, debug,
                                 per_gaussian_tau=True):
    lib = _lib.load()
    _require_cuda(means3D, "means3D")
    dev = means3D.device
    P = means3D.shape[0]
    H, W = dL_dout_color.shape[1], dL_dout_color.shape[2]
    sh = _prep(sh, dev, "sh")
    M = 0 if sh is None else sh.shape[1]
    f = dict(device=dev, dtype=_F32)
    dL_dmeans3D = torch.empty((P, 3), **f)
    dL_dmeans2D = torch.empty((P, 3), **f)
    dL_dcolors = torch.empty((P, 3), **f)
    dL_ddepths = torch.empty((P, 1), **f)
    dL_dconic = torch.empty((P, 2, 2), **f)
    dL_dopacity = torch.empty((P, 1), **f)
    dL_dcov3D = torch.empty((P, 6), **f)
    dL_dsh = torch.empty((P, M, 3), **f)
    dL_dscales = torch.empty((P, 3), **f)
    dL_drotations = torch.empty((P, 4), **f)
    dL_dtau = torch.empty((P, 6), **f) if per_gaussian_tau else None
    dL_dtau_sum = torch.zeros((6,), **f)
    if P == 0:
        return (dL_dmeans2D, dL_dcolors, dL_dopacity, dL_dmeans3D, dL_dcov3D, dL_dsh, dL_dscales, dL_drotations,
                dL_dtau, dL_dtau_sum, dL_dconic, dL_ddepths)
    means3D = _prep(means3D, dev, "means3D")
    colors = _prep(colors, dev, "colors")
    scales = _prep(scales, dev, "scales")
    rotations = _prep(rotations, dev, "rotations")
    cov3D_precomp = _prep(cov3D_precomp, dev, "cov3D")
    background = _prep(background, dev, "bg")
    viewmatrix = _prep(viewmatrix, dev, "viewmatrix")
    projmatrix = _prep(projmatrix, dev, "projmatrix")
    projmatrix_raw = _prep(projmatrix_raw, dev, "projmatrix_raw")
    campos = _prep(campos, dev, "campos")
    dL_dout_color = _prep(dL_dout_color, dev, "dL_dout_color")
    dL_dout_depths = _prep(dL_dout_depths, dev, "dL_dout_depths")
    st = _stream(dev)
    with torch.cuda.device(dev):
        _lib.check(lib.gsaj_rasterize_backward(
            P, int(degree), M, int(R), _ptr(background), W, H, _ptr(means3D), _ptr(sh), _ptr(colors), _ptr(scales),
            float(scale_modifier), _ptr(rotations), _ptr(cov3D_precomp), _ptr(viewmatrix), _ptr(projmatrix),
            _ptr(projmatrix_raw), _ptr(campos), float(tan_fovx), float(tan_fovy), radii.data_ptr(),
            geomBuffer.data_ptr(), binningBuffer.data_ptr(), imageBuffer.data_ptr(), _ptr(dL_dout_color),
            _ptr(dL_dout_depths), dL_dmeans2D.data_ptr(), dL_dconic.data_ptr(), dL_dopacity.data_ptr(),
            dL_dcolors.data_ptr(), dL_ddepths.data_ptr(), dL_dmeans3D.data_ptr(), dL_dcov3D.data_ptr(),
            _ptr(dL_dsh), _ptr(dL_dscales) if scales is not None else None,
            _ptr(dL_drotations) if rotations is not None else None,
            dL_dtau.data_ptr() if dL_dtau is not None else None, dL_dtau_sum.data_ptr(), st), "gsaj_rasterize_backward")
        if debug:
            torch.cuda.synchronize(dev)
    if scales is None:
        dL_dscales.zero_()
        dL_drotations.zero_()
    return (dL_dmeans2D, dL_dcolors, dL_dopacity, dL_dmeans3D, dL_dcov3D, dL_dsh, dL_dscales, dL_drotations, dL_dtau,
            dL_dtau_sum, dL_dconic, dL_ddepths)


def mark_visible(means3D, viewmatrix, projmatrix):
    lib = _lib.load()
    _require_cuda(means3D, "means3D")
    dev = means3D.device
    P = means3D.shape[0]
    present = torch.zeros((P,), device=dev, dtype=torch.bool)
    if P != 0:
        means3D = _prep(means3D, dev, "means3D")
        viewmatrix = _prep(viewmatrix, dev, "viewmatrix")
        projmatrix = _prep(projmatrix, dev, "projmatrix")
        with torch.cuda.device(dev):
            _lib.check(lib.gsaj_mark_visible(P, _ptr(means3D), _ptr(viewmatrix), _ptr(projmatrix), present.data_ptr(),
                                             _stream(dev)), "gsaj_mark_visible")
    return present


def debug_export(P, R, W, H, geomBuffer, binningBuffer, imageBuffer):
    lib = _lib.load()
    dev = geomBuffer.device
    tiles = ((W + 15) // 16) * ((H + 15) // 16)
    f = dict(device=dev, dtype=_F32)
    out = dict(
        means2D=torch.zeros((P, 2), **f), depths=torch.zeros((P,), **f), cov3D=torch.zeros((P, 6), **f),
        conic_opacity=torch.zeros((P, 4), **f), rgb=torch.zeros((P, 3), **f),
        clamped=torch.zeros((P, 3), device=dev, dtype=torch.uint8),
        tiles_touched=torch.zeros((P,), device=dev, dtype=torch.int32),
        point_list=torch.zeros((max(R, 1),), device=dev, dtype=torch.int32),
        ranges=torch.zeros((tiles, 2), device=dev, dtype=torch.int32), final_T=torch.zeros((H, W), **f),
        n_contrib=torch.zeros((H, W), device=dev, dtype=torch.int32))
    with torch.cuda.device(dev):
        _lib.check(lib.gsaj_debug_export(
            P, R, W, H, geomBuffer.data_ptr(), binningBuffer.data_ptr(), imageBuffer.data_ptr(),
            out["means2D"].data_ptr(), out["depths"].data_ptr(), out["cov3D"].data_ptr(),
            out["conic_opacity"].data_ptr(), out["rgb"].data_ptr(), out["clamped"].data_ptr(),
            out["tiles_touched"].data_ptr(), out["point_list"].data_ptr(), out["ranges"].data_ptr(),
            out["final_T"].data_ptr(), out["n_contrib"].data_ptr(), _stream(dev)), "gsaj_debug_export")
    out["point_list"] = out["point_list"][:R]
    return out


STAGE_NAMES = ("preprocess,scan_blocks,emit_keys,sort,ranges_records,render_fwd,render_bwd,gaussian_bwd,tau_finalize,"
               "dense_bwd,dense_reduce,scatter_instances,tile_sort_records,gather_sums").split(",")


class profile_stages:

    def __init__(self, max_records=4096):
        self.max_records = max_records
        self.ms, self.launches = {}, {}

    def __enter__(self):
        _lib.check(_lib.load().gsaj_profile_begin(self.max_records), "gsaj_profile_begin")
        return self

    def __exit__(self, *exc):
        n = len(STAGE_NAMES)
        ms = (ctypes.c_float * n)()
        cnt = (ctypes.c_int * n)()
        _lib.check(_lib.load().gsaj_profile_end(ctypes.cast(ms, ctypes.c_void_p), ctypes.cast(cnt, ctypes.c_void_p)),
                   "gsaj_profile_end")
        self.ms = {k: float(ms[i]) for i, k in enumerate(STAGE_NAMES)}
        self.launches = {k: int(cnt[i]) for i, k in enumerate(STAGE_NAMES)}
        return False


FWD_RECORDS_FP16 = 1


def _fwd_flags(record_bits):
    if record_bits not in (16, 32):
        raise ValueError("record_bits must be 16 or 32, got %r" % (record_bits,))
    return FWD_RECORDS_FP16 if record_bits == 16 else 0


class ArenaWatch:

    def __init__(self, img, K, img_stride, counters_offset, every=4, grow_at=0.75):
        self.K, self.every, self.grow_at = int(K), int(every), float(grow_at)
        i32 = img.view(torch.int32)
        self.dev_counters = torch.as_strided(i32, (self.K, 4), (img_stride // 4, 1), counters_offset // 4)
        self.host = torch.zeros((self.K, 4), dtype=torch.int32).pin_memory()
        self.event = torch.cuda.Event()
        self.pending, self.calls = False, 0
        self.grown = 0
        with torch.cuda.device(img.device):
            self.host.copy_(self.dev_counters, non_blocking=True)
            self.event.record()
            self.event.synchronize()

    def post(self):
        self.calls += 1
        if self.pending or self.calls % self.every or torch.cuda.is_current_stream_capturing():
            return
        self.host.copy_(self.dev_counters, non_blocking=True)
        self.event.record()
        self.pending = True

    def poll(self):
        if not self.pending or torch.cuda.is_current_stream_capturing() or not self.event.query():
            return None
        self.pending = False
        return int(self.host[:, 0].max()), int(self.host[:, 2].max())


class FrameContext:

    def __init__(self, P, W, H, M, device, has_scales=True, per_gaussian_tau=False, grad_slots=1, n_keyframes=0,
                 keyframe=0, record_bits=32):
        lib = _lib.load()
        self.flags = _fwd_flags(record_bits)
        self.lib, self.P, self.W, self.H, self.M, self.dev = lib, P, W, H, M, torch.device(device)
        f = dict(device=self.dev, dtype=_F32)
        byte = dict(device=self.dev, dtype=torch.uint8)
        self.color = torch.zeros((3, H, W), **f)
        self.depth = torch.zeros((1, H, W), **f)
        self.opacity = torch.zeros((1, H, W), **f)
        self.radii = torch.zeros((P,), device=self.dev, dtype=torch.int32)
        self.n_touched = torch.zeros((P,), device=self.dev, dtype=torch.int32)
        self.geom = torch.empty(lib.gsaj_geom_workspace_bytes(P), **byte)
        self.img = torch.zeros(lib.gsaj_image_workspace_bytes(W, H), **byte)
        self.binning = torch.empty(0, **byte)
        self.R = 0
        self.capacity = 0
        self.tile_list_capacity = 0
        self.watch = ArenaWatch(self.img, 1, self.img.numel(), self.abort_flag_ptr() - 16 - self.img.data_ptr())
        self.auto_grow = os.environ.get("GSAJ_ARENA_WATCH", "1") != "0"
        from .keyframe_shard import bucket_numel, bucket_views
        self.buckets, self.slots = [], []
        for _ in range(max(1, grad_slots)):
            bucket = torch.zeros(bucket_numel(P, M, has_scales, n_keyframes), **f)
            v = bucket_views(bucket, P, M, has_scales, n_keyframes)
            self.buckets.append(bucket)
            self.slots.append(dict(
                mean2D=torch.zeros((P, 3), **f), conic=torch.zeros((P, 2, 2), **f), opacity=v["opacity"],
                color=torch.zeros((P, 3), **f), depth=torch.zeros((P, 1), **f), mean3D=v["mean3D"],
                cov3D=v["cov3D"] if not has_scales else torch.zeros((P, 6), **f), sh=v["sh"].view(P, M, 3),
                scale=v.get("scale"), rot=v.get("rot"),
                tau=torch.zeros((P, 6), **f) if per_gaussian_tau else None,
                tau_sum=v["tau_all"][keyframe] if n_keyframes else torch.zeros((6,), **f),
                tau_all=v.get("tau_all")))
        self.bucket, self.g = self.buckets[0], self.slots[0]

    def set_tile_band(self, tile_row_begin, tile_row_end):
        _lib.check(self.lib.gsaj_set_tile_band(self.W, self.H, self.img.data_ptr(), int(tile_row_begin), int(tile_row_end),
                                               _stream(self.dev)), "gsaj_set_tile_band")
        self.band = (int(tile_row_begin), int(tile_row_end))

    def abort_flag_ptr(self):
        return self.lib.gsaj_forward_abort_flag(self.W, self.H, self.img.data_ptr())

    def abort_flag_tensor(self):
        off = self.abort_flag_ptr() - self.img.data_ptr()
        return self.img[off:off + 4].view(torch.int32)

    def _grow_ahead(self):
        seen = self.watch.poll() if self.auto_grow else None
        if seen is None:
            return
        R, longest = seen
        if R > self.watch.grow_at * self.capacity:
            self.capacity = int(R * 1.5) + 1024
            self.binning = torch.empty(self.lib.gsaj_binning_workspace_bytes(self.capacity), device=self.dev, dtype=torch.uint8)
            self.watch.grown += 1
        if longest > self.tile_list_capacity:
            self.tile_list_capacity = min(SORT_CAP, int(1.1 * longest) + 1)

    def _ensure_binning(self, R):
        need = self.lib.gsaj_binning_workspace_bytes(R)
        if self.binning.numel() < need:
            self.capacity = int(R * 1.5) + 1024
            self.binning = torch.empty(self.lib.gsaj_binning_workspace_bytes(self.capacity), device=self.dev,
                                       dtype=torch.uint8)

    def status(self):
        n = ctypes.c_int(0)
        _lib.check(self.lib.gsaj_forward_aborted_count(self.W, self.H, self.img.data_ptr(), _stream(self.dev),
                                                       ctypes.byref(n)), "gsaj_forward_aborted_count")
        R, mt = ctypes.c_int(0), ctypes.c_int(0)
        _lib.check(self.lib.gsaj_forward_num_rendered(self.W, self.H, self.img.data_ptr(), _stream(self.dev),
                                                      ctypes.byref(R), ctypes.byref(mt)), "gsaj_forward_num_rendered")
        self.true_R = R.value
        if n.value:
            raise _lib.GsajError("%d asynchronous forward(s) were aborted on the device (binning arena too small for the frame's "
                                 "instances); run forward(sync=True) to re-size" % n.value)
        return R.value, mt.value

    def forward(self, bg, means3D, opacities, viewmatrix, projmatrix, campos, tanfovx, tanfovy, sh_degree=0, shs=None,
                colors_precomp=None, scales=None, rotations=None, cov3D_precomp=None, scale_modifier=1.0, sync=True):
        with torch.cuda.device(self.dev):
            return self._forward(bg, means3D, opacities, viewmatrix, projmatrix, campos, tanfovx, tanfovy, sh_degree, shs, colors_precomp,
                                 scales, rotations, cov3D_precomp, scale_modifier, sync)

    def _forward(self, bg, means3D, opacities, viewmatrix, projmatrix, campos, tanfovx, tanfovy, sh_degree, shs, colors_precomp, scales,
                 rotations, cov3D_precomp, scale_modifier, sync):
        lib, st = self.lib, _stream(self.dev)
        if not sync and self.capacity > 0:
            self._grow_ahead()
            _lib.check(lib.gsaj_rasterize_forward_async(
                self.P, int(sh_degree), self.M, _ptr(bg), self.W, self.H, _ptr(means3D), _ptr(shs), _ptr(colors_precomp),
                _ptr(opacities), _ptr(scales), float(scale_modifier), _ptr(rotations), _ptr(cov3D_precomp),
                _ptr(viewmatrix), _ptr(projmatrix), _ptr(campos), float(tanfovx), float(tanfovy), 0,
                self.color.data_ptr(), self.depth.data_ptr(), self.opacity.data_ptr(), self.radii.data_ptr(),
                self.n_touched.data_ptr(), self.geom.data_ptr(), self.binning.data_ptr(), self.binning.numel(),
                self.capacity, self.tile_list_capacity, self.img.data_ptr(), self.flags, st), "gsaj_rasterize_forward_async")
            self.R = self.capacity
            if self.auto_grow:
                self.watch.post()
            return self.R
        _lib.check(lib.gsaj_forward_preprocess(
            self.P, int(sh_degree), self.M, self.W, self.H, _ptr(means3D), _ptr(shs), _ptr(colors_precomp),
            _ptr(opacities), _ptr(scales), float(scale_modifier), _ptr(rotations), _ptr(cov3D_precomp), _ptr(viewmatrix),
            _ptr(projmatrix), _ptr(campos), float(tanfovx), float(tanfovy), 0, self.radii.data_ptr(),
            self.n_touched.data_ptr(), self.geom.data_ptr(), self.img.data_ptr(), st), "gsaj_forward_preprocess")
        R, mt = ctypes.c_int(0), ctypes.c_int(0)
        _lib.check(lib.gsaj_forward_num_rendered(self.W, self.H, self.img.data_ptr(), st, ctypes.byref(R), ctypes.byref(mt)),
                   "gsaj_forward_num_rendered")
        self.R, self.max_tile_list = R.value, mt.value
        self.tile_list_capacity = min(SORT_CAP, max(self.tile_list_capacity, int(1.1 * self.max_tile_list) + 1, 256))
        self._ensure_binning(self.R)
        self.true_R = self.R
        _lib.check(lib.gsaj_forward_render(
            self.P, self.R, -1 if FORCE_CHUNKED_SORT else self.max_tile_list, self.W, self.H, _ptr(bg), _ptr(colors_precomp), self.radii.data_ptr(), self.geom.data_ptr(),
            self.binning.data_ptr(), self.binning.numel(), self.img.data_ptr(), self.color.data_ptr(),
            self.depth.data_ptr(), self.opacity.data_ptr(), self.n_touched.data_ptr(), self.flags, st), "gsaj_forward_render")
        return self.R

    def forward_loss(self, loss, bg, means3D, opacities, viewmatrix, projmatrix, campos, tanfovx, tanfovy, sh_degree=0, shs=None,
                     colors_precomp=None, scales=None, rotations=None, cov3D_precomp=None, scale_modifier=1.0):
        if self.capacity <= 0:
            raise _lib.GsajError("forward_loss: size the arena with one synchronous forward() first")
        if not hasattr(self, "loss_ws"):
            self.loss_ws = torch.empty(self.lib.gsaj_fused_loss_workspace_bytes(self.W, self.H), device=self.dev, dtype=torch.uint8)
        with torch.cuda.device(self.dev):
            self._grow_ahead()
            _lib.check(self.lib.gsaj_rasterize_forward_loss(
                self.P, int(sh_degree), self.M, _ptr(bg), self.W, self.H, _ptr(means3D), _ptr(shs), _ptr(colors_precomp),
                _ptr(opacities), _ptr(scales), float(scale_modifier), _ptr(rotations), _ptr(cov3D_precomp),
                _ptr(viewmatrix), _ptr(projmatrix), _ptr(campos), float(tanfovx), float(tanfovy), 0,
                self.color.data_ptr(), self.depth.data_ptr(), self.opacity.data_ptr(), self.radii.data_ptr(),
                self.n_touched.data_ptr(), self.geom.data_ptr(), self.binning.data_ptr(), self.binning.numel(),
                self.capacity, self.tile_list_capacity, self.img.data_ptr(), self.flags, int(loss["flags"]), float(loss["alpha"]),
                float(loss["rgb_boundary_threshold"]), _ptr(loss["gt_color"]), _ptr(loss.get("gt_depth")), _ptr(loss.get("grad_mask")),
                _ptr(loss.get("exposure_a")), _ptr(loss.get("exposure_b")), loss["scalars"].data_ptr(), self.loss_ws.data_ptr(),
                _stream(self.dev)), "gsaj_rasterize_forward_loss")
            if self.auto_grow:
                self.watch.post()
        self.R = self.capacity
        return self.R

    def backward_loss(self, loss, bg, means3D, viewmatrix, projmatrix, projmatrix_raw, campos, tanfovx, tanfovy, sh_degree=0, shs=None,
                      colors_precomp=None, scales=None, rotations=None, cov3D_precomp=None, scale_modifier=1.0, slot=0,
                      pose_only=False):
        g = self.slots[slot]
        if g["tau_all"] is not None:
            g["tau_all"].zero_()
        with torch.cuda.device(self.dev):
            _lib.check(self.lib.gsaj_rasterize_backward_loss(
                self.P, int(sh_degree), self.M, self.R, _ptr(bg), self.W, self.H, _ptr(means3D), _ptr(shs),
                _ptr(colors_precomp), _ptr(scales), float(scale_modifier), _ptr(rotations), _ptr(cov3D_precomp),
                _ptr(viewmatrix), _ptr(projmatrix), _ptr(projmatrix_raw), _ptr(campos), float(tanfovx), float(tanfovy),
                self.radii.data_ptr(), self.geom.data_ptr(), self.binning.data_ptr(), self.img.data_ptr(), int(loss["flags"]),
                float(loss["alpha"]), float(loss["rgb_boundary_threshold"]), self.color.data_ptr(), self.depth.data_ptr(),
                self.opacity.data_ptr(), _ptr(loss["gt_color"]), _ptr(loss.get("gt_depth")), _ptr(loss.get("grad_mask")),
                _ptr(loss.get("exposure_a")), _ptr(loss.get("exposure_b")), *([None] * 10 if pose_only else [
                    g["mean2D"].data_ptr(), g["conic"].data_ptr(), g["opacity"].data_ptr(), g["color"].data_ptr(),
                    g["depth"].data_ptr(), g["mean3D"].data_ptr(), g["cov3D"].data_ptr(), _ptr(g["sh"]), _ptr(g["scale"]),
                    _ptr(g["rot"])]), _ptr(g["tau"]), g["tau_sum"].data_ptr(), _stream(self.dev)), "gsaj_rasterize_backward_loss")
        return g

    def backward(self, bg, means3D, viewmatrix, projmatrix, projmatrix_raw, campos, tanfovx, tanfovy, dL_dcolor, dL_ddepth,
                 sh_degree=0, shs=None, colors_precomp=None, scales=None, rotations=None, cov3D_precomp=None,
                 scale_modifier=1.0, slot=0, pose_only=False):
        g = self.slots[slot]
        if g["tau_all"] is not None:
            g["tau_all"].zero_()
        with torch.cuda.device(self.dev):
            self._backward(g, bg, means3D, viewmatrix, projmatrix, projmatrix_raw, campos, tanfovx, tanfovy, dL_dcolor, dL_ddepth, sh_degree,
                           shs, colors_precomp, scales, rotations, cov3D_precomp, scale_modifier, pose_only)
        return g

    def _backward(self, g, bg, means3D, viewmatrix, projmatrix, projmatrix_raw, campos, tanfovx, tanfovy, dL_dcolor, dL_ddepth, sh_degree,
                  shs, colors_precomp, scales, rotations, cov3D_precomp, scale_modifier, pose_only):
        _lib.check(self.lib.gsaj_rasterize_backward(
            self.P, int(sh_degree), self.M, self.R, _ptr(bg), self.W, self.H, _ptr(means3D), _ptr(shs),
            _ptr(colors_precomp), _ptr(scales), float(scale_modifier), _ptr(rotations), _ptr(cov3D_precomp),
            _ptr(viewmatrix), _ptr(projmatrix), _ptr(projmatrix_raw), _ptr(campos), float(tanfovx), float(tanfovy),
            self.radii.data_ptr(), self.geom.data_ptr(), self.binning.data_ptr(), self.img.data_ptr(), _ptr(dL_dcolor),
            _ptr(dL_ddepth), *([None] * 10 if pose_only else [
                g["mean2D"].data_ptr(), g["conic"].data_ptr(), g["opacity"].data_ptr(), g["color"].data_ptr(),
                g["depth"].data_ptr(), g["mean3D"].data_ptr(), g["cov3D"].data_ptr(), _ptr(g["sh"]), _ptr(g["scale"]),
                _ptr(g["rot"])]), _ptr(g["tau"]), g["tau_sum"].data_ptr(), _stream(self.dev)),
            "gsaj_rasterize_backward")
        return g

    def interactions(self):
        dbg = debug_export(self.P, self.R, self.W, self.H, self.geom, self.binning, self.img)
        return int(dbg["n_contrib"].to(torch.int64).sum().item())


class BatchContext:

    def __init__(self, K, P, W, H, M, device, has_scales=True, record_bits=32, per_gaussian_tau=False, grad_slots=1,
                 n_windows=1, window=0, streams=1):
        from .keyframe_shard import bucket_numel, bucket_views
        lib = _lib.load()
        self.lib, self.K, self.P, self.W, self.H, self.M, self.dev = lib, int(K), int(P), int(W), int(H), int(M), torch.device(device)
        self.flags = _fwd_flags(record_bits)
        f = dict(device=self.dev, dtype=_F32)
        byte = dict(device=self.dev, dtype=torch.uint8)
        self.color = torch.zeros((K, 3, H, W), **f)
        self.depth = torch.zeros((K, 1, H, W), **f)
        self.opacity = torch.zeros((K, 1, H, W), **f)
        self.radii = torch.zeros((K, P), device=self.dev, dtype=torch.int32)
        self.n_touched = torch.zeros((K, P), device=self.dev, dtype=torch.int32)
        self.geom_stride = lib.gsaj_geom_workspace_bytes(P)
        self.img_stride = lib.gsaj_image_workspace_bytes(W, H)
        self.geom = torch.empty(K * self.geom_stride, **byte)
        self.img = torch.zeros(K * self.img_stride, **byte)
        self.binning = torch.empty(0, **byte)
        self.capacity, self.tile_list_capacity, self.bin_stride = 0, 0, 0
        self.watch = ArenaWatch(self.img, self.K, self.img_stride, lib.gsaj_forward_abort_flag(W, H, self.img.data_ptr()) - 16 - self.img.data_ptr())
        self.auto_grow = os.environ.get("GSAJ_ARENA_WATCH", "1") != "0"
        self.buckets, self.slots = [], []
        for _ in range(max(1, grad_slots)):
            bucket = torch.zeros(bucket_numel(P, M, has_scales, K * n_windows), **f)
            v = bucket_views(bucket, P, M, has_scales, K * n_windows)
            self.buckets.append(bucket)
            self.slots.append(dict(mean2D=torch.zeros((K, P, 3), **f), opacity=v["opacity"], mean3D=v["mean3D"],
                                   cov3D=v["cov3D"] if not has_scales else torch.zeros((P, 6), **f), sh=v["sh"].view(P, M, 3),
                                   scale=v.get("scale"), rot=v.get("rot"), tau=torch.zeros((K, P, 6), **f) if per_gaussian_tau else None,
                                   tau_all=v["tau_all"][window * K:(window + 1) * K], tau_every_window=v["tau_all"] if n_windows > 1 else None))
        self.bucket, self.g = self.buckets[0], self.slots[0]
        if streams >= 2 and K >= 2:
            k0 = (K + 1) // 2
            self.groups = [(0, k0, None), (k0, K - k0, torch.cuda.Stream(self.dev))]
        else:
            self.groups = [(0, K, None)]

    def _size(self, capacity):
        self.capacity = int(capacity)
        self.bin_stride = self.lib.gsaj_binning_workspace_bytes(self.capacity)
        self.binning = torch.empty(self.K * self.bin_stride, device=self.dev, dtype=torch.uint8)

    def set_tile_band(self, tile_row_begin, tile_row_end, views=None):
        for v in (range(self.K) if views is None else views):
            _lib.check(self.lib.gsaj_set_tile_band(self.W, self.H, self.img.data_ptr() + int(v) * self.img_stride, int(tile_row_begin),
                                                   int(tile_row_end), _stream(self.dev)), "gsaj_set_tile_band")

    def status(self):
        out, st = [], _stream(self.dev)
        for v in range(self.K):
            R, mt = ctypes.c_int(0), ctypes.c_int(0)
            rc = self.lib.gsaj_forward_num_rendered(self.W, self.H, self.img.data_ptr() + v * self.img_stride, st, ctypes.byref(R), ctypes.byref(mt))
            if rc not in (0, -3):
                _lib.check(rc, "gsaj_forward_num_rendered")
            out.append((R.value, mt.value, rc == -3))
        return out

    def abort_flags(self):
        return self.lib.gsaj_forward_abort_flag(self.W, self.H, self.img.data_ptr()), self.img_stride

    def clear_aborts(self):
        total, st = 0, _stream(self.dev)
        for v in range(self.K):
            n = ctypes.c_int(0)
            _lib.check(self.lib.gsaj_forward_aborted_count(self.W, self.H, self.img.data_ptr() + v * self.img_stride, st, ctypes.byref(n)),
                       "gsaj_forward_aborted_count")
            total += n.value
        return total

    def _fork(self):
        cur = torch.cuda.current_stream(self.dev)
        for _, _, st in self.groups:
            if st is not None:
                st.wait_stream(cur)
        return cur

    def _join(self, cur):
        for _, _, st in self.groups:
            if st is not None:
                cur.wait_stream(st)

    def _launch(self, bg, means3D, opacities, viewmatrices, projmatrices, campos, tanfovx, tanfovy, sh_degree, shs, colors_precomp, scales,
                rotations, cov3D_precomp, scale_modifier):
        HW, P = self.H * self.W, self.P
        cur = self._fork()
        for v0, kv, st in self.groups:
            stream = cur if st is None else st
            _lib.check(self.lib.gsaj_rasterize_forward_batch(
                kv, P, int(sh_degree), self.M, _ptr(bg), self.W, self.H, _ptr(means3D), _ptr(shs), _ptr(colors_precomp),
                _ptr(opacities), _ptr(scales), float(scale_modifier), _ptr(rotations), _ptr(cov3D_precomp),
                viewmatrices.data_ptr() + 64 * v0, projmatrices.data_ptr() + 64 * v0, None if campos is None else campos.data_ptr() + 12 * v0,
                float(tanfovx), float(tanfovy), 0, self.color.data_ptr() + 12 * HW * v0, self.depth.data_ptr() + 4 * HW * v0,
                self.opacity.data_ptr() + 4 * HW * v0, self.radii.data_ptr() + 4 * P * v0, self.n_touched.data_ptr() + 4 * P * v0,
                self.geom.data_ptr() + self.geom_stride * v0, self.binning.data_ptr() + self.bin_stride * v0, self.bin_stride * kv,
                self.capacity, self.tile_list_capacity, self.img.data_ptr() + self.img_stride * v0, self.flags, stream.cuda_stream),
                "gsaj_rasterize_forward_batch")
        self._join(cur)

    def forward(self, bg, means3D, opacities, viewmatrices, projmatrices, campos, tanfovx, tanfovy, sh_degree=0, shs=None,
                colors_precomp=None, scales=None, rotations=None, cov3D_precomp=None, scale_modifier=1.0, sync=True):
        a = (bg, means3D, opacities, viewmatrices, projmatrices, campos, tanfovx, tanfovy, sh_degree, shs, colors_precomp, scales,
             rotations, cov3D_precomp, scale_modifier)
        if self.capacity == 0:
            self._size(max(4096, 12 * self.P))
        elif not sync and self.auto_grow:
            seen = self.watch.poll()
            if seen is not None:
                if seen[0] > self.watch.grow_at * self.capacity:
                    self._size(int(1.5 * seen[0]) + 1024)
                    self.watch.grown += 1
                if seen[1] > self.tile_list_capacity > 0:
                    self.tile_list_capacity = min(SORT_CAP, int(1.1 * seen[1]) + 1)
        self._launch(*a)
        if not sync:
            if self.auto_grow:
                self.watch.post()
            return None
        st = self.status()
        if any(ab for _, _, ab in st):
            self._size(int(1.5 * max(r for r, _, _ in st)) + 1024)
            self.tile_list_capacity = 0
            self.clear_aborts()
            self._launch(*a)
            st = self.status()
            if any(ab for _, _, ab in st):
                raise _lib.GsajError("the batch was aborted again after re-sizing the arena to %d instances per view: %r" % (self.capacity, st))
        if self.auto_grow and max(r for r, _, _ in st) > self.watch.grow_at * self.capacity:
            self._size(int(1.5 * max(r for r, _, _ in st)) + 1024)
            self._launch(*a)
            st = self.status()
        self.tile_list_capacity = min(SORT_CAP, max(self.tile_list_capacity, int(1.1 * max(m for _, m, _ in st)) + 1, 256))
        return st

    def backward(self, bg, means3D, viewmatrices, projmatrices, projmatrix_raw, campos, tanfovx, tanfovy, dL_dcolor, dL_ddepth,
                 sh_degree=0, shs=None, colors_precomp=None, scales=None, rotations=None, cov3D_precomp=None, scale_modifier=1.0, slot=0,
                 split=False):
        g = self.slots[slot]
        if g["tau_every_window"] is not None:
            g["tau_every_window"].zero_()
        HW, P = self.H * self.W, self.P

        def call(v0, kv, stream, flags):
            _lib.check(self.lib.gsaj_rasterize_backward_batch(
                kv, P, int(sh_degree), self.M, self.capacity, _ptr(bg), self.W, self.H, _ptr(means3D), _ptr(shs),
                _ptr(colors_precomp), _ptr(scales), float(scale_modifier), _ptr(rotations), _ptr(cov3D_precomp),
                viewmatrices.data_ptr() + 64 * v0, projmatrices.data_ptr() + 64 * v0, _ptr(projmatrix_raw),
                None if campos is None else campos.data_ptr() + 12 * v0, float(tanfovx), float(tanfovy), self.radii.data_ptr() + 4 * P * v0,
                self.geom.data_ptr() + self.geom_stride * v0, self.binning.data_ptr() + self.bin_stride * v0,
                self.img.data_ptr() + self.img_stride * v0, dL_dcolor.data_ptr() + 12 * HW * v0, dL_ddepth.data_ptr() + 4 * HW * v0,
                g["mean2D"].data_ptr() + 12 * P * v0, None, g["opacity"].data_ptr(), None, None, g["mean3D"].data_ptr(),
                g["cov3D"].data_ptr(), _ptr(g["sh"]), _ptr(g["scale"]), _ptr(g["rot"]),
                None if g["tau"] is None else g["tau"].data_ptr() + 24 * P * v0, g["tau_all"].data_ptr() + 24 * v0, flags,
                stream.cuda_stream), "gsaj_rasterize_backward_batch")

        cur = self._fork()
        if len(self.groups) == 1:
            if split:
                call(0, self.K, cur, 2)
                call(0, self.K, cur, 4)
            else:
                call(0, self.K, cur, 0)
            return g
        for v0, kv, st in self.groups:
            call(v0, kv, cur if st is None else st, 2)
        self._join(cur)
        for i, (v0, kv, st) in enumerate(self.groups):
            call(v0, kv, cur, 4 | (1 if i > 0 else 0))
        return g

    def view_sums(self, v, stored=False):
        out = torch.zeros((self.P, 12), device=self.dev, dtype=_F32)
        v = int(v)
        if stored:
            _lib.check(self.lib.gsaj_debug_export_view_sums(self.P, self.geom.data_ptr() + v * self.geom_stride, out.data_ptr(),
                                                            _stream(self.dev)), "gsaj_debug_export_view_sums")
            return out
        _lib.check(self.lib.gsaj_debug_export_view_sums_gather(
            self.P, self.capacity, self.W, self.H, self.geom.data_ptr() + v * self.geom_stride, self.binning.data_ptr() + v * self.bin_stride,
            self.img.data_ptr() + v * self.img_stride, out.data_ptr(), _stream(self.dev)), "gsaj_debug_export_view_sums_gather")
        return out

    def interactions(self):
        total = 0
        for v in range(self.K):
            n = torch.zeros((self.H, self.W), device=self.dev, dtype=torch.int32)
            _lib.check(self.lib.gsaj_debug_export(self.P, 0, self.W, self.H, None, None, self.img.data_ptr() + v * self.img_stride,
                                                  None, None, None, None, None, None, None, None, None, None, n.data_ptr(),
                                                  _stream(self.dev)), "gsaj_debug_export")
            total += int(n.to(torch.int64).sum().item())
        return total
```

include/gsaj.h:

```cpp
#ifndef GSAJ_H_INCLUDED
#define GSAJ_H_INCLUDED

#include <stddef.h>
#include <stdint.h>

#ifdef __cplusplus
extern "C" {
#endif

#define GSAJ_OK 0
#define GSAJ_ERR_INVALID_ARGUMENT (-1)
#define GSAJ_ERR_HIP (-2)
#define GSAJ_ERR_WORKSPACE_TOO_SMALL (-3)
#define GSAJ_ERR_PREFILTERED_CULLED (-4)

#define GSAJ_TILE 16
#define GSAJ_NUM_CHANNELS 3

const char *gsaj_last_error(void);
int gsaj_version(void);

size_t gsaj_geom_workspace_bytes(int P);
size_t gsaj_image_workspace_bytes(int W, int H);
size_t gsaj_binning_workspace_bytes(int R);

#define GSAJ_FWD_RECORDS_FP16 1

int gsaj_forward_preprocess(int P, int D, int M, int W, int H,
                            const float *means3D , const float *shs ,
                            const float *colors_precomp , const float *opacities ,
                            const float *scales , float scale_modifier,
                            const float *rotations , const float *cov3D_precomp ,
                            const float *viewmatrix , const float *projmatrix ,
                            const float *campos , float tanfovx, float tanfovy, int prefiltered,
                            int *radii , int *n_touched ,
                            void *geom_ws , void *image_ws , void *stream);
int gsaj_forward_num_rendered(int W, int H, const void *image_ws, void *stream, int *num_rendered ,
                              int *max_tile_list );
int gsaj_forward_render(int P, int R, int max_tile_list , int W, int H,
                        const float *bg ,
                        const float *colors_precomp , const int *radii ,
                        void *geom_ws, void *binning_ws, size_t binning_ws_bytes, void *image_ws,
                        float *out_color, float *out_depth, float *out_opacity, int *n_touched,
                        int flags , void *stream);

int gsaj_rasterize_forward(int P, int D, int M, const float *bg, int W, int H,
                           const float *means3D, const float *shs, const float *colors_precomp,
                           const float *opacities, const float *scales, float scale_modifier,
                           const float *rotations, const float *cov3D_precomp,
                           const float *viewmatrix, const float *projmatrix, const float *campos,
                           float tanfovx, float tanfovy, int prefiltered,
                           float *out_color, float *out_depth, float *out_opacity, int *radii, int *n_touched,
                           void *geom_ws, void *binning_ws, size_t binning_ws_bytes, void *image_ws,
                           int *num_rendered_out , int flags , void *stream);

int gsaj_rasterize_forward_async(int P, int D, int M, const float *bg, int W, int H,
                                 const float *means3D, const float *shs, const float *colors_precomp,
                                 const float *opacities, const float *scales, float scale_modifier,
                                 const float *rotations, const float *cov3D_precomp,
                                 const float *viewmatrix, const float *projmatrix, const float *campos,
                                 float tanfovx, float tanfovy, int prefiltered,
                                 float *out_color, float *out_depth, float *out_opacity, int *radii, int *n_touched,
                                 void *geom_ws, void *binning_ws, size_t binning_ws_bytes, int capacity, int tile_list_capacity,
                                 void *image_ws, int flags , void *stream);
int gsaj_forward_aborted_count(int W, int H, void *image_ws, void *stream, int *count );

const uint32_t *gsaj_forward_abort_flag(int W, int H, void *image_ws);

int gsaj_set_tile_band(int W, int H, void *image_ws, int tile_row_begin, int tile_row_end, void *stream);
int gsaj_forward_preprocess_cap(int P, int D, int M, int W, int H,
                                const float *means3D, const float *shs, const float *colors_precomp,
                                const float *opacities, const float *scales, float scale_modifier,
                                const float *rotations, const float *cov3D_precomp,
                                const float *viewmatrix, const float *projmatrix, const float *campos,
                                float tanfovx, float tanfovy, int prefiltered, int *radii, int *n_touched,
                                void *geom_ws, void *image_ws, int capacity, int tile_list_capacity, void *stream);

int gsaj_rasterize_backward(int P, int D, int M, int R, const float *bg, int W, int H,
                            const float *means3D, const float *shs, const float *colors_precomp,
                            const float *scales, float scale_modifier, const float *rotations,
                            const float *cov3D_precomp, const float *viewmatrix, const float *projmatrix,
                            const float *projmatrix_raw, const float *campos, float tanfovx, float tanfovy,
                            const int *radii, void *geom_ws, void *binning_ws, void *image_ws,
                            const float *dL_dpix, const float *dL_dpix_depth,
                            float *dL_dmean2D, float *dL_dconic, float *dL_dopacity, float *dL_dcolor,
                            float *dL_ddepth, float *dL_dmean3D, float *dL_dcov3D, float *dL_dsh,
                            float *dL_dscale, float *dL_drot, float *dL_dtau, float *dL_dtau_sum, void *stream);

int gsaj_rasterize_forward_batch(int K, int P, int D, int M, const float *bg, int W, int H, const float *means3D,
                                 const float *shs, const float *colors_precomp, const float *opacities, const float *scales,
                                 float scale_modifier, const float *rotations, const float *cov3D_precomp,
                                 const float *viewmatrices, const float *projmatrices, const float *campos, float tanfovx,
                                 float tanfovy, int prefiltered, float *out_color, float *out_depth, float *out_opacity,
                                 int *radii, int *n_touched, void *geom_ws, void *binning_ws, size_t binning_ws_bytes,
                                 int capacity, int tile_list_capacity, void *image_ws, int flags , void *stream);
int gsaj_rasterize_backward_batch(int K, int P, int D, int M, int capacity, const float *bg, int W, int H,
                                  const float *means3D, const float *shs, const float *colors_precomp, const float *scales,
                                  float scale_modifier, const float *rotations, const float *cov3D_precomp,
                                  const float *viewmatrices, const float *projmatrices, const float *projmatrix_raw,
                                  const float *campos, float tanfovx, float tanfovy, const int *radii, void *geom_ws,
                                  void *binning_ws, void *image_ws, const float *dL_dpix, const float *dL_dpix_depth,
                                  float *dL_dmean2D, float *dL_dconic, float *dL_dopacity, float *dL_dcolor, float *dL_ddepth,
                                  float *dL_dmean3D, float *dL_dcov3D, float *dL_dsh, float *dL_dscale, float *dL_drot,
                                  float *dL_dtau, float *dL_dtau_sum, int flags , void *stream);
#define GSAJ_BWD_ACCUMULATE 1
#define GSAJ_BWD_ONLY_COMPOSITE 2
#define GSAJ_BWD_ONLY_CHAIN 4

int gsaj_mark_visible(int P, const float *means3D, const float *viewmatrix, const float *projmatrix,
                      uint8_t *present , void *stream);

int gsaj_debug_export(int P, int R, int W, int H, const void *geom_ws, const void *binning_ws, const void *image_ws,
                      float *means2D, float *depths, float *cov3D, float *conic_opacity, float *rgb, uint8_t *clamped,
                      uint32_t *tiles_touched, uint32_t *point_list, uint32_t *ranges, float *final_T,
                      uint32_t *n_contrib, void *stream);

int gsaj_debug_export_view_sums(int P, const void *geom_ws, float *sums , void *stream);
int gsaj_debug_export_view_sums_gather(int P, int capacity, int W, int H, void *geom_ws, void *binning_ws, void *image_ws,
                                       float *sums , void *stream);

#define GSAJ_NUM_STAGES 14
#define GSAJ_STAGE_NAMES "preprocess,scan_blocks,emit_keys,sort,ranges_records,render_fwd,render_bwd,gaussian_bwd,tau_finalize,dense_bwd,dense_reduce,scatter_instances,tile_sort_records,gather_sums"
int gsaj_profile_begin(int max_records);
int gsaj_profile_end(float *stage_ms , int *stage_launches );

#define GSAJ_LOSS_TRACKING 1
#define GSAJ_LOSS_MONOCULAR 2
#define GSAJ_LOSS_NO_EXPOSURE 4
#define GSAJ_LOSS_COMPUTE_LOSS 8
size_t gsaj_loss_workspace_bytes(int W, int H);
int gsaj_loss_seeds(int W, int H, int flags, float alpha, float rgb_boundary_threshold, const float *color,
                    const float *depth, const float *opacity, const float *gt_color, const float *gt_depth,
                    const uint8_t *grad_mask, const float *exposure_a, const float *exposure_b, float *dL_dcolor,
                    float *dL_ddepth, float *dL_dopacity, float *out_scalars, void *loss_ws, void *stream);

size_t gsaj_fused_loss_workspace_bytes(int W, int H);
int gsaj_rasterize_forward_loss(int P, int D, int M, const float *bg, int W, int H, const float *means3D, const float *shs,
                                const float *colors_precomp, const float *opacities, const float *scales, float scale_modifier,
                                const float *rotations, const float *cov3D_precomp, const float *viewmatrix,
                                const float *projmatrix, const float *campos, float tanfovx, float tanfovy, int prefiltered,
                                float *out_color, float *out_depth, float *out_opacity, int *radii, int *n_touched, void *geom_ws,
                                void *binning_ws, size_t binning_ws_bytes, int capacity, int tile_list_capacity, void *image_ws,
                                int flags , int loss_flags , float alpha,
                                float rgb_boundary_threshold, const float *gt_color ,
                                const float *gt_depth , const uint8_t *grad_mask ,
                                const float *exposure_a, const float *exposure_b ,
                                float *out_scalars , void *loss_ws, void *stream);
int gsaj_rasterize_backward_loss(int P, int D, int M, int R, const float *bg, int W, int H, const float *means3D, const float *shs,
                                 const float *colors_precomp, const float *scales, float scale_modifier, const float *rotations,
                                 const float *cov3D_precomp, const float *viewmatrix, const float *projmatrix,
                                 const float *projmatrix_raw, const float *campos, float tanfovx, float tanfovy, const int *radii,
                                 void *geom_ws, void *binning_ws, void *image_ws, int loss_flags, float alpha,
                                 float rgb_boundary_threshold, const float *color, const float *depth, const float *opacity,
                                 const float *gt_color, const float *gt_depth, const uint8_t *grad_mask, const float *exposure_a,
                                 const float *exposure_b, float *dL_dmean2D, float *dL_dconic, float *dL_dopacity, float *dL_dcolor,
                                 float *dL_ddepth, float *dL_dmean3D, float *dL_dcov3D, float *dL_dsh, float *dL_dscale,
                                 float *dL_drot, float *dL_dtau, float *dL_dtau_sum, void *stream);

int gsaj_loss_seeds_batch(int K, int W, int H, int flags, float alpha, float rgb_boundary_threshold, const float *color,
                          const float *depth, const float *opacity, const float *gt_color, const float *gt_depth,
                          const uint8_t *grad_mask, const float *exposure_a, const float *exposure_b, float *dL_dcolor,
                          float *dL_ddepth, float *dL_dopacity, float *out_scalars, void *loss_ws, void *stream);

size_t gsaj_isotropic_workspace_bytes(int P);
int gsaj_isotropic_loss(int P, int C, float weight, const float *scales, float *dL_dscales, int accumulate, float *out_loss,
                        void *iso_ws, void *stream);

size_t gsaj_ssim_workspace_bytes(int N, int C, int W, int H);
int gsaj_ssim_forward(int N, int C, int W, int H, const float *img, const float *gt, float *ssim_out, float *ssim_map,
                      void *ssim_ws, void *stream);
int gsaj_ssim_backward(int N, int C, int W, int H, const float *img, const float *gt, const float *dL_dssim, float *dL_dimg,
                       void *ssim_ws, void *stream);
size_t gsaj_refine_loss_workspace_bytes(int W, int H);
int gsaj_refine_loss_seeds(int W, int H, float lambda_dssim, const float *image, const float *gt, float *dL_dcolor,
                           float *out_scalars, void *ws, void *stream);

int gsaj_densification_stats(int K, int P, const float *dL_dmean2D, const int *radii, const int *n_touched,
                             float *xyz_gradient_accum, float *denom, float *max_radii2D, int *n_obs, void *stream);

#define GSAJ_POSE_STATE_FLOATS 80
int gsaj_pose_state_floats(void);
int gsaj_pose_adam_step(const float *dL_dtau, const float *dL_dexposure, float lr_rot, float lr_trans, float lr_exp_a,
                        float lr_exp_b, float beta1, float beta2, float eps, float converged_threshold,
                        const float *projection_matrix, float *pose_state, const uint32_t *skip, void *stream);

int gsaj_pose_adam_step_batch(int K, const float *dL_dtau, const float *dL_dexposure, const uint8_t *active, float lr_rot,
                              float lr_trans, float lr_exp_a, float lr_exp_b, float beta1, float beta2, float eps,
                              float converged_threshold, const float *projection_matrix, float *pose_states, const uint32_t *skip,
                              size_t skip_stride_bytes, void *stream);

size_t gsaj_dist2_workspace_bytes(int P);
int gsaj_dist2(int P, const float *points, float *mean_dists, void *knn_ws, void *stream);
int gsaj_debug_dist2_order(int P, void *knn_ws, uint32_t *codes_sorted, uint32_t *idx_sorted, void *stream);

size_t gsaj_seed_workspace_bytes(int W, int H);
int gsaj_depth_stats(int W, int H, const float *depth, const float *opacity , float opacity_min,
                     const uint8_t *mask , const float *gt_image , float rgb_threshold,
                     float *out_stats , uint8_t *out_valid , void *seed_ws, void *stream);
int gsaj_keyframe_depth_prior(int W, int H, const float *depth, const float *opacity, const float *gt_image, float rgb_threshold,
                              const float *noise , float *out_depth , float *out_stats ,
                              void *seed_ws, void *stream);
int gsaj_seed_select(int W, int H, const float *depth, const float *gt_image , float rgb_threshold, float depth_trunc,
                     double downsample_factor, uint32_t seed, void *seed_ws, void *stream);
int gsaj_seed_count(const void *seed_ws, void *stream, int *n_valid , int *m );
int gsaj_seed_gaussians(int m, int W, int H, const float *depth, const float *image, const float *exposure_ab ,
                        const float *w2c , double fx, double fy, double cx, double cy, float point_size, int adaptive,
                        int sh_coeffs, int isotropic, float *xyz, float *f_dc, float *f_rest, float *scaling, float *rotation,
                        float *opacity, void *seed_ws, void *knn_ws, void *stream);
int gsaj_debug_seed_pixels(int W, int H, int m, const void *seed_ws, uint32_t *pixels, void *stream);

size_t gsaj_grad_mask_workspace_bytes(int W, int H);
int gsaj_grad_intensity(int W, int H, const float *image, float *out_intensity , void *stream);
int gsaj_grad_mask(int W, int H, const float *image, float edge_threshold, int blocks, uint8_t *out_mask_u8 ,
                   float *out_mask_f32 , void *ws, void *stream);

#define GSAJ_COVIS_MAX_SLOTS 32
int gsaj_covis_pack(int K, int P, const int *n_touched , const int *slots , uint32_t clear_mask,
                    uint32_t *words , void *stream);
int gsaj_covis_query(int P, const uint32_t *words, const int *cur_n_touched , int query_slot,
                     uint32_t slot_mask, int *out , void *stream);
int gsaj_covis_prune_mask(int P, const uint32_t *words, uint32_t window_mask, const int *unique_kfIDs ,
                          int kf_id_min, int max_obs, uint8_t *to_prune , int *n_obs ,
                          int *n_pruned , void *stream);

size_t gsaj_dense_workspace_bytes(int N, int W, int H);
#define GSAJ_DENSE_NAIVE_GUARDS 1
#define GSAJ_DENSE_NORMALISED_COORDS 2
int gsaj_dense_backward(int N, int W, int H, const float *means2D, const float *covs2D, const float *colors,
                        const float *depths, const float *opac, const float *seed_color, const float *seed_depth,
                        float *grad_mu, float *grad_Sigma, float *grad_depth, float *grad_color,
                        void *dense_ws, int flags, const double *intrinsics , void *stream);
size_t gsaj_dense_project_workspace_bytes(int N);
int gsaj_dense_project(int N, int sh_coeffs, int sh_degree, int W, int H, const float *means3D, const float *cov3D,
                       const float *shs, const float *viewmatrix, const float *projmatrix, const float *campos, double fx,
                       double fy, int *order, double *mean2D, double *cov2D, double *color, double *color_raw, double *depth,
                       void *project_ws, void *stream);
int gsaj_dense_render(int N, int W, int H, const float *means2D, const float *covs2D, const float *colors,
                      const float *depths, const float *opac, float *out_color, float *out_depth, void *stream);
int gsaj_pose_jacobians(int N, const double *T_cw , const double *mu_w, const double *cov3D, double fx,
                        double fy, int W, int H, double *dmu_dtau, double *dcov_dtau, void *stream);
int gsaj_dense_tau(int N, int sh_coeffs, int sh_degree, const int *order, const float *grad_mu,
                   const float *grad_Sigma, const float *grad_depth, const float *grad_color,
                   const double *dmu_dtau, const double *dcov_dtau, const double *mu_w, const double *T_cw,
                   const double *campos, const double *shs , double *dL_dtau ,
                   double *parts , void *stream);

#ifdef __cplusplus
}
#endif
#endif
```

Before: 698.0 billion interactions/s.

## Record per-quadrant taken flags in forward and compact live list for backward

The forward render now writes a per-instance byte mask showing which 8x8 quadrants actually composited each Gaussian, using wave-mask ballots instead of per-lane bools. Backward first sweeps that mask to build a compacted list of (id, position|quadrant bits) in the reused keys buffer. It then walks only those live entries, replacing the per-round quadrant_relevant test with a bit lookup. This adds forward stores, a prepass and a bigger workspace in exchange for fewer iterations and less ellipse testing in backward. Forward waves_per_eu is also raised, and a debug export path is added.

```diff
diff --git a/gs-slam-analytica_jacobian_amd/csrc/api.hip b/gs-slam-analytica_jacobian_amd/csrc/api.hip
--- a/gs-slam-analytica_jacobian_amd/csrc/api.hip
+++ b/gs-slam-analytica_jacobian_amd/csrc/api.hip
@@ -616,6 +616,22 @@
   return GSAJ_OK;
 }
 
+int gsaj_debug_export_taken(int R, int W, int H, const void *binning_ws, const void *image_ws, uint32_t *taken, uint8_t *reached,
+                            void *stream) {
+  if (R <= 0 || W <= 0 || H <= 0 || !binning_ws || !image_ws) {
+    gsaj_set_error("gsaj_debug_export_taken: invalid argument");
+    return GSAJ_ERR_INVALID_ARGUMENT;
+  }
+  hipStream_t s = (hipStream_t)stream;
+  BinWS b;
+  bin_carve(align_base(const_cast<void *>(binning_ws)), (size_t)R, &b);
+  ImageWS im;
+  image_carve(align_base(const_cast<void *>(image_ws)), W, H, &im);
+  if (reached) GSAJ_HIP_CHECK(hipMemcpyAsync(reached, b.reached, (size_t)R, hipMemcpyDeviceToDevice, s));
+  if (taken) return launch_export_taken(W, H, (W + TILE - 1) / TILE, (H + TILE - 1) / TILE, b, im, taken, s);
+  return GSAJ_OK;
+}
+
 int gsaj_debug_export_view_sums(int P, const void *geom_ws, float *sums, void *stream) {
   if (P <= 0 || !geom_ws || !sums) {
     gsaj_set_error("gsaj_debug_export_view_sums: invalid argument");
diff --git a/gs-slam-analytica_jacobian_amd/csrc/gsaj_common.h b/gs-slam-analytica_jacobian_amd/csrc/gsaj_common.h
--- a/gs-slam-analytica_jacobian_amd/csrc/gsaj_common.h
+++ b/gs-slam-analytica_jacobian_amd/csrc/gsaj_common.h
@@ -102,6 +102,7 @@
   uint32_t *point_list;
   float4 *inst_grad;
   uint8_t *reached;
+  uint32_t *taken;
 };
 
 struct ViewStrides {
@@ -139,6 +140,7 @@
   CARVE(point_list, uint32_t, Rn);
   CARVE(inst_grad, float4, Rn * REC_F4);
   CARVE(reached, uint8_t, Rn);
+  CARVE(taken, uint32_t, Rn);
   return off;
 }
 #undef CARVE
@@ -191,6 +193,7 @@
 int launch_render_backward(int R, int W, int H, int grid_x, int grid_y, const float *bg, const GeomWS &g, const BinWS &b,
                            const ImageWS &im, const float *dL_dpix, const float *dL_dpix_depth, int views, ViewStrides vs,
                            hipStream_t s, const FusedLoss *fl = nullptr);
+int launch_export_taken(int W, int H, int grid_x, int grid_y, const BinWS &b, const ImageWS &im, uint32_t *out, hipStream_t s);
 struct BwdParams {
   int P, D, M, W, H;
   const float *means3D, *shs, *scales, *rotations, *cov3Ds;
@@ -282,6 +285,11 @@
 }
 __device__ __forceinline__ uint32_t gsaj_load_u32_global(const uint32_t *src) {
   return *reinterpret_cast<const __attribute__((address_space(1))) uint32_t *>((unsigned long long)src);
+}
+__device__ __forceinline__ uint2 gsaj_load_u64_device(const uint2 *src) {
+  const unsigned long long v = __hip_atomic_load(reinterpret_cast<const __attribute__((address_space(1))) unsigned long long *>((unsigned long long)src),
+                                                 __ATOMIC_RELAXED, __HIP_MEMORY_SCOPE_AGENT);
+  return make_uint2((uint32_t)v, (uint32_t)(v >> 32));
 }
 __device__ __forceinline__ uint4 gsaj_coherent_load_x4(const void *src) {
   uint4 v;
diff --git a/gs-slam-analytica_jacobian_amd/csrc/render_bwd.hip b/gs-slam-analytica_jacobian_amd/csrc/render_bwd.hip
--- a/gs-slam-analytica_jacobian_amd/csrc/render_bwd.hip
+++ b/gs-slam-analytica_jacobian_amd/csrc/render_bwd.hip
@@ -18,7 +18,8 @@
 
 template <bool LOSS>
 __global__ __launch_bounds__(256) __attribute__((amdgpu_waves_per_eu(5, 5))) void k_render_bwd(int W, int H, int gx, ImageWS im,
-                                                    const uint32_t *__restrict__ point_list, GeomWS g,
+                                                    const uint32_t *__restrict__ point_list, const uint32_t *__restrict__ taken,
+                                                    uint2 *__restrict__ live, GeomWS g,
                                                     const float *__restrict__ bg,
                                                     const float *__restrict__ dL_dpix,
                                                     const float *__restrict__ dL_dpix_depth,
@@ -28,6 +29,8 @@
     const size_t view = blockIdx.y, HWv = (size_t)H * W;
     im = image_view(im, view * vs.image);
     point_list = gsaj_shift(point_list, view * vs.bin);
+    taken = gsaj_shift(taken, view * vs.bin);
+    live = gsaj_shift(live, view * vs.bin);
     g = geom_view(g, view * vs.geom);
     inst_grad = gsaj_shift(inst_grad, view * vs.bin);
     reached = gsaj_shift(reached, view * vs.bin);
@@ -44,6 +47,8 @@
   __shared__ float4 seed_all[4 * 64];
   __shared__ uint32_t wave_max[4];
   __shared__ uint32_t blk_first[BWD_ROUND];
+  __shared__ uint32_t ent_pos[2][BWD_ROUND];
+  __shared__ uint32_t sweep_cnt[2][4];
   if (counters[4]) return;
   GSAJ_TRACE_BEGIN(bwd)
   const int tid = threadIdx.x, wave = tid >> 6, lane = tid & 63;
@@ -63,6 +68,7 @@
   const float T_final = inside ? final_T[pid] : 0.f;
   float T = T_final;
   const uint32_t last = inside ? n_contrib[pid] : 0u;
+  const uint32_t last4 = last << 4;
   float gC0 = 0.f, gC1 = 0.f, gC2 = 0.f, gD = 0.f;
   if (inside) {
     if (LOSS) {
@@ -88,21 +94,46 @@
   for (int o = 32; o > 0; o >>= 1) wmax = max(wmax, (uint32_t)__shfl_xor((int)wmax, o));
   if (lane == 0) wave_max[wave] = wmax;
   __syncthreads();
-  const uint32_t bmax = max(max(wave_max[0], wave_max[1]), max(wave_max[2], wave_max[3]));
+  const uint32_t wm0 = (uint32_t)__builtin_amdgcn_readfirstlane((int)wave_max[0]), wm1 = (uint32_t)__builtin_amdgcn_readfirstlane((int)wave_max[1]);
+  const uint32_t wm2 = (uint32_t)__builtin_amdgcn_readfirstlane((int)wave_max[2]), wm3 = (uint32_t)__builtin_amdgcn_readfirstlane((int)wave_max[3]);
+  const uint32_t bmax = min(max(max(wm0, wm1), max(wm2, wm3)), range.y - range.x);
+
+  uint2 *__restrict__ seg = live + range.x;
+  uint32_t nlive = 0u;
+  for (uint32_t p0 = 0u, it = 0u; p0 < bmax; p0 += 256u, it ^= 1u) {
+    const uint32_t p = p0 + (uint32_t)tid;
+    const bool in = p < bmax;
+    const uint32_t word = gsaj_load_u32_global(taken + range.x + (in ? p : 0u));
+    const uint32_t id = gsaj_load_u32_global(point_list + range.x + (in ? p : 0u));
+    const uint32_t keep = (p < wm0 ? 0x1u : 0u) | (p < wm1 ? 0x100u : 0u) | (p < wm2 ? 0x10000u : 0u) | (p < wm3 ? 0x1000000u : 0u);
+    const uint32_t qb = (((word & keep) * 0x00204081u) >> 21) & 0xfu;
+    const unsigned long long bal = __builtin_amdgcn_ballot_w64(in && qb != 0u);
+    if (lane == 0) sweep_cnt[it][wave] = (uint32_t)__popcll(bal);
+    __syncthreads();
+    const uint32_t c0 = sweep_cnt[it][0], c1 = sweep_cnt[it][1], c2 = sweep_cnt[it][2], c3 = sweep_cnt[it][3];
+    if (in && qb != 0u) {
+      const uint32_t before = (wave > 0 ? c0 : 0u) + (wave > 1 ? c1 : 0u) + (wave > 2 ? c2 : 0u);
+      const uint32_t at = nlive + before + __builtin_amdgcn_mbcnt_hi((uint32_t)(bal >> 32), __builtin_amdgcn_mbcnt_lo((uint32_t)bal, 0u));
+      seg[at] = make_uint2(id, (p << 4) | qb);
+    }
+    nlive = (uint32_t)__builtin_amdgcn_readfirstlane((int)(nlive + c0 + c1 + c2 + c3));
+  }
+  asm volatile("s_waitcnt vmcnt(0)" ::: "memory");
+  __syncthreads();
 
   float accS = 0.f;
 
   const int p2_slot = lane & (SLOTS - 1), p2_row = lane >> 3;
   const float p2_py = qy0 + (float)p2_row;
 
-  uint32_t hi = (uint32_t)__builtin_amdgcn_readfirstlane((int)(range.x + bmax));
+  uint32_t hi = nlive;
   const bool rec16 = counters[7] != 0u;
   const int part = __builtin_amdgcn_readfirstlane(wave), e = lane;
-  auto round_lo = [&](uint32_t h) { return (h - range.x > BWD_ROUND) ? h - BWD_ROUND : range.x; };
-  auto load_id = [&](uint32_t l, uint32_t h) -> uint32_t {
+  auto round_lo = [&](uint32_t h) { return h > BWD_ROUND ? h - BWD_ROUND : 0u; };
+  auto load_ent = [&](uint32_t l, uint32_t h) -> uint2 {
     const bool has = e < BWD_ROUND && l + (uint32_t)e < h;
-    const uint32_t v = gsaj_load_u32_global(point_list + (has ? l + (uint32_t)e : range.x));
-    return has ? v : 0xffffffffu;
+    const uint2 v = gsaj_load_u64_device(seg + (has ? l + (uint32_t)e : 0u));
+    return has ? v : make_uint2(0xffffffffu, 0u);
   };
   const char *piece_base;
   uint32_t piece_stride;
@@ -115,13 +146,15 @@
     const size_t off = piece_stride ? (size_t)i * piece_stride : (size_t)(i / PRE_BLOCK) * 4u;
     return gsaj_load_f4_unaligned(piece_base + off);
   };
-  uint32_t id_cur = 0xffffffffu, id_nxt = 0xffffffffu;
+  uint2 ent_nxt = make_uint2(0xffffffffu, 0u);
   float4 piece = make_float4(0.f, 0.f, 0.f, 0.f);
-  if (hi > range.x) {
+  uint32_t par = 0u;
+  if (hi > 0u) {
     const uint32_t lo0 = round_lo(hi);
-    id_cur = load_id(lo0, hi);
-    id_nxt = load_id(round_lo(lo0), lo0);
-    piece = load_piece(id_cur);
+    const uint2 ent = load_ent(lo0, hi);
+    ent_nxt = load_ent(round_lo(lo0), lo0);
+    if (part == 2 && e < BWD_ROUND) ent_pos[0][e] = ent.y;
+    piece = load_piece(ent.x);
   }
 
 #ifdef GSAJ_BLOCK_TRACE
@@ -129,7 +162,7 @@
   unsigned tr_flushes = 0u, tr_slots = 0u;
   unsigned long long pht_ = wall_clock64();
 #endif
-  while (hi > range.x) {
+  while (hi > 0u) {
     BWD_PH(6)
     const uint32_t lo = round_lo(hi);
     const int n = (int)(hi - lo);
@@ -165,9 +198,10 @@
     }
     {
       const uint32_t lo2 = round_lo(lo);
-      id_cur = id_nxt;
-      id_nxt = load_id(round_lo(lo2), lo2);
-      piece = load_piece(id_cur);
+      const uint2 ent = ent_nxt;
+      ent_nxt = load_ent(round_lo(lo2), lo2);
+      if (part == 2 && e < BWD_ROUND) ent_pos[par ^ 1u][e] = ent.y;
+      piece = load_piece(ent.x);
     }
     {
       float4 *z = reinterpret_cast<float4 *>(acc);
@@ -177,14 +211,9 @@
     __syncthreads();
     BWD_PH(1)
 
-    const uint32_t first_idx = (uint32_t)__builtin_amdgcn_readfirstlane((int)(lo - range.x));
-    if (wmax > first_idx) {
-      bool rel = false;
-      if (lane < n && first_idx + (uint32_t)lane < wmax) {
-        const float4 q0 = rec[lane * REC_F4 + 0];
-        const float4 q1 = rec[lane * REC_F4 + 1];
-        rel = quadrant_relevant(q0.x, q0.y, (-2.0f / GSAJ_LOG2E) * q1.x, (-1.0f / GSAJ_LOG2E) * q1.y, (-2.0f / GSAJ_LOG2E) * q1.z, q1.w, qx0, qy0);
-      }
+    const uint32_t *pos_r = ent_pos[par];
+    {
+      const bool rel = lane < n && ((pos_r[min(lane, BWD_ROUND - 1)] >> wave) & 1u) != 0u;
       unsigned long long todo = __builtin_amdgcn_ballot_w64(rel);
       int nslot = 0;
       unsigned long long slot_pack = 0ull;
@@ -249,7 +278,7 @@
         float4 k = rec[jj * REC_F4 + 1], c = rec[jj * REC_F4 + 2];
         while (true) {
           const int j = jj;
-          const uint32_t idx = first_idx + (uint32_t)j;
+          const uint32_t idx4 = pos_r[j];
           const bool more = todo != 0ull;
           if (more) {
             jj = 63 - __builtin_clzll(todo);
@@ -260,7 +289,7 @@
           const float oG = k.w * __builtin_amdgcn_exp2f(p2);
           q01 = reinterpret_cast<const float2 *>(rec)[jj * (REC_F4 * 2)];
           k = rec[jj * REC_F4 + 1];
-          const bool valid = idx < last && p2 <= 0.0f && oG >= (1.0f / 255.0f);
+          const bool valid = idx4 < last4 && p2 <= 0.0f && oG >= (1.0f / 255.0f);
           float cg = __builtin_fmaf(c.x, gC0, __builtin_fmaf(c.y, gC1, __builtin_fmaf(c.z, gC2, c.w * gD)));
           asm volatile("" : "+v"(cg));
           c = rec[jj * REC_F4 + 2];
@@ -308,6 +337,7 @@
     __syncthreads();
     BWD_PH(5)
     hi = lo;
+    par ^= 1u;
   }
 #ifdef GSAJ_BLOCK_TRACE
   {
@@ -330,12 +360,38 @@
   {
     GsajProfScope ps(ST_RENDER_BWD, s);
     if (fl)
-      hipLaunchKernelGGL(k_render_bwd<true>, dim3(grid_x * grid_y, 1), dim3(256), 0, s, W, H, grid_x, im, b.point_list, g, bg, dL_dpix,
-                         dL_dpix_depth, b.inst_grad, b.reached, vs, *fl);
+      hipLaunchKernelGGL(k_render_bwd<true>, dim3(grid_x * grid_y, 1), dim3(256), 0, s, W, H, grid_x, im, b.point_list, b.taken, reinterpret_cast<uint2 *>(b.keys), g, bg,
+                         dL_dpix, dL_dpix_depth, b.inst_grad, b.reached, vs, *fl);
     else
-      hipLaunchKernelGGL(k_render_bwd<false>, dim3(grid_x * grid_y, views), dim3(256), 0, s, W, H, grid_x, im, b.point_list, g, bg, dL_dpix,
-                         dL_dpix_depth, b.inst_grad, b.reached, vs, FusedLoss{});
+      hipLaunchKernelGGL(k_render_bwd<false>, dim3(grid_x * grid_y, views), dim3(256), 0, s, W, H, grid_x, im, b.point_list, b.taken, reinterpret_cast<uint2 *>(b.keys), g, bg,
+                         dL_dpix, dL_dpix_depth, b.inst_grad, b.reached, vs, FusedLoss{});
   }
   GSAJ_HIP_CHECK(hipGetLastError());
   return GSAJ_OK;
 }
+
+__global__ __launch_bounds__(256) void k_export_taken(int W, int H, int gx, ImageWS im, const uint32_t *__restrict__ taken,
+                                                      uint32_t *__restrict__ out) {
+  __shared__ uint32_t wave_max[4];
+  if (im.counters[4]) return;
+  const int tid = threadIdx.x, wave = tid >> 6, lane = tid & 63;
+  const int tile = blockIdx.x, ty = tile / gx, tx = tile - ty * gx;
+  const int px = tx * TILE + (wave & 1) * 8 + (lane & 7), py = ty * TILE + (wave >> 1) * 8 + (lane >> 3);
+  uint32_t wmax = (px < W && py < H) ? im.n_contrib[(size_t)py * W + px] : 0u;
+#pragma unroll
+  for (int o = 32; o > 0; o >>= 1) wmax = max(wmax, (uint32_t)__shfl_xor((int)wmax, o));
+  if (lane == 0) wave_max[wave] = wmax;
+  __syncthreads();
+  const uint2 range = im.ranges[tile];
+  for (uint32_t p = (uint32_t)tid; p < range.y - range.x; p += 256u) {
+    const uint32_t keep = (p < wave_max[0] ? 0x1u : 0u) | (p < wave_max[1] ? 0x100u : 0u) | (p < wave_max[2] ? 0x10000u : 0u) |
+                          (p < wave_max[3] ? 0x1000000u : 0u);
+    out[range.x + p] = taken[range.x + p] & keep;
+  }
+}
+
+int launch_export_taken(int W, int H, int grid_x, int grid_y, const BinWS &b, const ImageWS &im, uint32_t *out, hipStream_t s) {
+  hipLaunchKernelGGL(k_export_taken, dim3(grid_x * grid_y), dim3(256), 0, s, W, H, grid_x, im, b.taken, out);
+  GSAJ_HIP_CHECK(hipGetLastError());
+  return GSAJ_OK;
+}
diff --git a/gs-slam-analytica_jacobian_amd/csrc/render_fwd.hip b/gs-slam-analytica_jacobian_amd/csrc/render_fwd.hip
--- a/gs-slam-analytica_jacobian_amd/csrc/render_fwd.hip
+++ b/gs-slam-analytica_jacobian_amd/csrc/render_fwd.hip
@@ -15,18 +15,20 @@
 GSAJ_TRACE_DEFINE(fwd)
 
 template <bool LOSS>
-__global__ __launch_bounds__(GSAJ_FWD_THREADS) __attribute__((amdgpu_waves_per_eu(5, 8))) void k_render_fwd(int W, int H, int gx, int tiles, int P, ImageWS im,
+__global__ __launch_bounds__(GSAJ_FWD_THREADS) __attribute__((amdgpu_waves_per_eu(6, 8))) void k_render_fwd(int W, int H, int gx, int tiles, int P, ImageWS im,
                                                     const float4 *__restrict__ splat, const float4 *__restrict__ splat16,
                                                     const float *__restrict__ bg,
                                                     float *__restrict__ out_color, float *__restrict__ out_depth,
                                                     float *__restrict__ out_opacity, int *__restrict__ n_touched,
-                                                    const uint32_t *__restrict__ point_list, ViewStrides vs, FusedLoss fl) {
+                                                    const uint32_t *__restrict__ point_list, uint32_t *__restrict__ taken,
+                                                    ViewStrides vs, FusedLoss fl) {
   {
     const size_t view = blockIdx.y, HWv = (size_t)H * W;
     im = image_view(im, view * vs.image);
     splat = gsaj_shift(splat, view * vs.geom);
     splat16 = gsaj_shift(splat16, view * vs.geom);
     point_list = gsaj_shift(point_list, view * vs.bin);
+    taken = gsaj_shift(taken, view * vs.bin);
     out_color += view * 3 * HWv;
     out_depth += view * HWv;
     out_opacity += view * HWv;
@@ -62,15 +64,25 @@
   const float qx0 = (float)(tx * TILE + (wave & 1) * 8), qy0 = (float)(ty * TILE + (wave >> 1) * 8);
   const uint2 range = ranges[tile];
 
-  bool done = !inside;
+  unsigned long long done_m = __builtin_amdgcn_ballot_w64(!inside);
   float T = 1.0f;
   uint32_t last = 0;
   bool counting = true;
 
+  auto sel = [](unsigned long long m, float a, float b) -> float {
+    float r;
+    asm("v_cndmask_b32_e64 %0, %1, %2, %3" : "=v"(r) : "v"(b), "v"(a), "s"(m));
+    return r;
+  };
+  auto sel0 = [](unsigned long long m, float a) -> float {
+    float r;
+    asm("v_cndmask_b32_e64 %0, 0, %1, %2" : "=v"(r) : "v"(a), "s"(m));
+    return r;
+  };
   v2f Crg = {0.f, 0.f}, Cbd = {0.f, 0.f};
   const v2f px2 = {pxf, pxf}, py2 = {pyf, pyf};
   auto composite2 = [&](const float4 p0, const float4 p1, const float4 p2, const float4 cA, const float4 cB, const float2 pos,
-                        float &T_afterA) {
+                        float &T_afterA, unsigned long long &okA, unsigned long long &okB) {
     const v2f dx = v2f{p0.x, p0.y} - px2, dy = v2f{p0.z, p0.w} - py2;
     const v2f t = v2f{p1.z, p1.w} * dy;
     const v2f u = v2f{p2.x, p2.y} * dy;
@@ -78,36 +90,36 @@
     const v2f oe = v2f{p2.z, p2.w} * v2f{__builtin_amdgcn_exp2f(pw.x), __builtin_amdgcn_exp2f(pw.y)};
     {
       const float alpha0 = fminf(0.99f, oe.x);
-      bool ok = !done && pw.x <= 0.0f && alpha0 >= (1.0f / 255.0f);
       const float tA = __builtin_fmaf(-alpha0, T, T);
-      const bool sat = ok && tA < 0.0001f;
-      done = done || sat;
-      ok = ok && !sat;
-      const float w = ok ? alpha0 * T : 0.f;
+      const unsigned long long pre = __builtin_amdgcn_ballot_w64(pw.x <= 0.0f) & __builtin_amdgcn_ballot_w64(alpha0 >= (1.0f / 255.0f)) & ~done_m;
+      const unsigned long long sat = pre & __builtin_amdgcn_ballot_w64(tA < 0.0001f);
+      done_m |= sat;
+      okA = pre & ~sat;
+      const float w = sel0(okA, alpha0 * T);
       const v2f w2 = {w, w};
       Crg = __builtin_elementwise_fma(v2f{cA.x, cA.y}, w2, Crg);
       Cbd = __builtin_elementwise_fma(v2f{cA.z, cA.w}, w2, Cbd);
-      T = ok ? tA : T;
-      last = ok ? __float_as_uint(pos.x) : last;
+      T = sel(okA, tA, T);
+      last = __float_as_uint(sel(okA, pos.x, __uint_as_float(last)));
       T_afterA = T;
     }
     {
       const float alpha0 = fminf(0.99f, oe.y);
-      bool ok = !done && pw.y <= 0.0f && alpha0 >= (1.0f / 255.0f);
       const float tB = __builtin_fmaf(-alpha0, T, T);
-      const bool sat = ok && tB < 0.0001f;
-      done = done || sat;
-      ok = ok && !sat;
-      const float w = ok ? alpha0 * T : 0.f;
+      const unsigned long long pre = __builtin_amdgcn_ballot_w64(pw.y <= 0.0f) & __builtin_amdgcn_ballot_w64(alpha0 >= (1.0f / 255.0f)) & ~done_m;
+      const unsigned long long sat = pre & __builtin_amdgcn_ballot_w64(tB < 0.0001f);
+      done_m |= sat;
+      okB = pre & ~sat;
+      const float w = sel0(okB, alpha0 * T);
       const v2f w2 = {w, w};
       Crg = __builtin_elementwise_fma(v2f{cB.x, cB.y}, w2, Crg);
       Cbd = __builtin_elementwise_fma(v2f{cB.z, cB.w}, w2, Cbd);
-      T = ok ? tB : T;
-      last = ok ? __float_as_uint(pos.y) : last;
+      T = sel(okB, tB, T);
+      last = __float_as_uint(sel(okB, pos.y, __uint_as_float(last)));
     }
   };
 
-  if (__builtin_amdgcn_ballot_w64(!done) != 0ull && range.x < range.y) {
+  if (~done_m != 0ull && range.x < range.y) {
     float4 q0, q1, q2;
     uint32_t id_cur = 0u, id_nxt = 0u;
     const bool rec16 = counters[7] != 0u;
@@ -158,16 +170,17 @@
         const int pb = (i >> 1) * FWD_PAIR_F4;
         const float4 c0 = rec[pb + 6], c1 = rec[pb + 7], c2 = rec[pb + 8], c3 = rec[pb + 9], c4 = rec[pb + 10];
         const float2 c5 = rec2[(pb + 11) * 2];
-        uint32_t pack = 0u;
+        uint32_t pack;
         {
-          const float T0 = T;
           float Ta;
-          composite2(a0, a1, a2, a3, a4, a5, Ta);
+          unsigned long long okA, okB;
+          composite2(a0, a1, a2, a3, a4, a5, Ta, okA, okB);
+          pack = (okA != 0ull ? 0x80u : 0u) | (okB != 0ull ? 0x8000u : 0u);
           if (counting) {
             const unsigned long long hB = __builtin_amdgcn_ballot_w64(T > 0.5f);
-            const uint32_t nA = (uint32_t)__popcll(__builtin_amdgcn_ballot_w64(Ta > 0.5f) & __builtin_amdgcn_ballot_w64(Ta < T0));
-            const uint32_t nB = (uint32_t)__popcll(hB & __builtin_amdgcn_ballot_w64(T < Ta));
-            pack = nA | (nB << 8);
+            const uint32_t nA = (uint32_t)__popcll(__builtin_amdgcn_ballot_w64(Ta > 0.5f) & okA);
+            const uint32_t nB = (uint32_t)__popcll(hB & okB);
+            pack |= nA | (nB << 8);
             counting = hB != 0ull;
           }
         }
@@ -175,36 +188,46 @@
         a0 = rec[pb + 12], a1 = rec[pb + 13], a2 = rec[pb + 14], a3 = rec[pb + 15], a4 = rec[pb + 16];
         a5 = rec2[(pb + 17) * 2];
         {
-          const float T0 = T;
           float Tc;
-          composite2(c0, c1, c2, c3, c4, c5, Tc);
+          unsigned long long okC, okD;
+          composite2(c0, c1, c2, c3, c4, c5, Tc, okC, okD);
+          pack |= (okC != 0ull ? 0x800000u : 0u) | (okD != 0ull ? 0x80000000u : 0u);
           if (counting) {
             const unsigned long long hD = __builtin_amdgcn_ballot_w64(T > 0.5f);
-            const uint32_t nC = (uint32_t)__popcll(__builtin_amdgcn_ballot_w64(Tc > 0.5f) & __builtin_amdgcn_ballot_w64(Tc < T0));
-            const uint32_t nD = (uint32_t)__popcll(hD & __builtin_amdgcn_ballot_w64(T < Tc));
+            const uint32_t nC = (uint32_t)__popcll(__builtin_amdgcn_ballot_w64(Tc > 0.5f) & okC);
+            const uint32_t nD = (uint32_t)__popcll(hD & okD);
             pack |= (nC << 16) | (nD << 24);
             counting = hD != 0ull;
           }
         }
         cnt4 = ((lane >> 2) == (i >> 2)) ? pack : cnt4;
-        if (__builtin_amdgcn_ballot_w64(!done) == 0ull) {
+        if (~done_m == 0ull) {
           wave_done = true;
           break;
         }
       }
-      const int cnt = (int)((cnt4 >> (8 * (lane & 3))) & 0xffu);
+      const uint32_t mine = (cnt4 >> (8 * (lane & 3))) & 0xffu;
+      const int cnt = (int)(mine & 0x7fu);
       if (lane < nrel && cnt > 0) {
         const uint32_t id = __float_as_uint(recf[(lane >> 1) * FWD_PAIR_F4 * 4 + 22 + (lane & 1)]);
         atomicAdd(&n_touched[id], cnt);
       }
+      const int slot = __builtin_amdgcn_mbcnt_hi((uint32_t)(todo >> 32), __builtin_amdgcn_mbcnt_lo((uint32_t)todo, 0u));
+      const uint32_t took = (uint32_t)__shfl((int)mine, slot) >> 7;
+      if (lane < m) {
+        reinterpret_cast<uint8_t *>(taken + base)[(uint32_t)(lane * 4 + wave)] = rel ? (uint8_t)took : (uint8_t)0;
+      }
       __builtin_amdgcn_wave_barrier();
       if (wave_done) break;
     }
   }
 
   const float Cr = Crg.x, Cg = Crg.y, Cb = Cbd.x, Dp = Cbd.y;
+  int lane_e = lane;
+  asm volatile("" : "+v"(lane_e));
+  const int px_e = tx * TILE + (wave & 1) * 8 + (lane_e & 7), py_e = ty * TILE + (wave >> 1) * 8 + (lane_e >> 3);
   if (inside) {
-    const size_t pid = (size_t)py * W + px;
+    const size_t pid = (size_t)py_e * W + px_e;
     const size_t HW = (size_t)H * W;
     final_T[pid] = T;
     n_contrib[pid] = last;
@@ -217,7 +240,7 @@
   if (LOSS) {
     float s4[4] = {0.f, 0.f, 0.f, 0.f};
     if (inside) {
-      const size_t pid = (size_t)py * W + px, HW = (size_t)H * W;
+      const size_t pid = (size_t)py_e * W + px_e, HW = (size_t)H * W;
       const LossConsts L = loss_consts(fl.flags, fl.alpha, fl.rgb_thr, fl.exp_a, fl.exp_b, HW, 1.f);
       const bool mask = fl.grad_mask ? fl.grad_mask[pid] != 0 : true;
       const float gd = L.mono ? 0.f : fl.gt_depth[pid];
@@ -250,10 +273,10 @@
     const unsigned nblk = FWD_WAVES == 1 ? (unsigned)((tiles + 7) / 8) * 32u : (unsigned)tiles;
     if (fl)
       hipLaunchKernelGGL(k_render_fwd<true>, dim3(nblk, 1), dim3(GSAJ_FWD_THREADS), 0, s, W, H, grid_x, tiles, P, im, g.splat, g.splat16, bg,
-                         out_color, out_depth, out_opacity, n_touched, b.point_list, vs, *fl);
+                         out_color, out_depth, out_opacity, n_touched, b.point_list, b.taken, vs, *fl);
     else
       hipLaunchKernelGGL(k_render_fwd<false>, dim3(nblk, views), dim3(GSAJ_FWD_THREADS), 0, s, W, H, grid_x, tiles, P, im, g.splat, g.splat16,
-                         bg, out_color, out_depth, out_opacity, n_touched, b.point_list, vs, FusedLoss{});
+                         bg, out_color, out_depth, out_opacity, n_touched, b.point_list, b.taken, vs, FusedLoss{});
   }
   GSAJ_HIP_CHECK(hipGetLastError());
   return GSAJ_OK;
diff --git a/gs-slam-analytica_jacobian_amd/gsaj/_lib.py b/gs-slam-analytica_jacobian_amd/gsaj/_lib.py
--- a/gs-slam-analytica_jacobian_amd/gsaj/_lib.py
+++ b/gs-slam-analytica_jacobian_amd/gsaj/_lib.py
@@ -43,6 +43,7 @@
                                         c_float, c_float, P, P, P, P, P, P] + [P] * 12 + [P]),
     "gsaj_mark_visible": (c_int, [c_int, P, P, P, P, P]),
     "gsaj_debug_export": (c_int, [c_int] * 4 + [P] * 3 + [P] * 11 + [P]),
+    "gsaj_debug_export_taken": (c_int, [c_int, c_int, c_int, P, P, P, P, P]),
     "gsaj_debug_export_view_sums": (c_int, [c_int, P, P, P]),
     "gsaj_debug_export_view_sums_gather": (c_int, [c_int, c_int, c_int, c_int, P, P, P, P, P]),
     "gsaj_profile_begin": (c_int, [c_int]),
diff --git a/gs-slam-analytica_jacobian_amd/gsaj/rasterizer.py b/gs-slam-analytica_jacobian_amd/gsaj/rasterizer.py
--- a/gs-slam-analytica_jacobian_amd/gsaj/rasterizer.py
+++ b/gs-slam-analytica_jacobian_amd/gsaj/rasterizer.py
@@ -192,6 +192,17 @@
     return out
 
 
+def debug_export_taken(R, W, H, binningBuffer, imageBuffer):
+    lib = _lib.load()
+    dev = binningBuffer.device
+    taken = torch.zeros((max(R, 1),), device=dev, dtype=torch.int32)
+    reached = torch.zeros((max(R, 1),), device=dev, dtype=torch.uint8)
+    with torch.cuda.device(dev):
+        _lib.check(lib.gsaj_debug_export_taken(R, W, H, binningBuffer.data_ptr(), imageBuffer.data_ptr(), taken.data_ptr(),
+                                               reached.data_ptr(), _stream(dev)), "gsaj_debug_export_taken")
+    return taken[:R], reached[:R]
+
+
 STAGE_NAMES = ("preprocess,scan_blocks,emit_keys,sort,ranges_records,render_fwd,render_bwd,gaussian_bwd,tau_finalize,"
                "dense_bwd,dense_reduce,scatter_instances,tile_sort_records,gather_sums").split(",")
 
diff --git a/include/gsaj.h b/include/gsaj.h
--- a/include/gsaj.h
+++ b/include/gsaj.h
@@ -114,6 +114,9 @@
                       float *means2D, float *depths, float *cov3D, float *conic_opacity, float *rgb, uint8_t *clamped,
                       uint32_t *tiles_touched, uint32_t *point_list, uint32_t *ranges, float *final_T,
                       uint32_t *n_contrib, void *stream);
+
+int gsaj_debug_export_taken(int R, int W, int H, const void *binning_ws, const void *image_ws, uint32_t *taken ,
+                            uint8_t *reached , void *stream);
 
 int gsaj_debug_export_view_sums(int P, const void *geom_ws, float *sums , void *stream);
 int gsaj_debug_export_view_sums_gather(int P, int capacity, int W, int H, void *geom_ws, void *binning_ws, void *image_ws,
```

After: 733.2 billion interactions/s (median of 6 runs). +5.0%, better.
